# andrewdalpino/UltraZoom

Measured on AMD Instinct MI355X. Metric: upscaled MPix/sec, MewZoom-4X 1080p bf16 batched inference, higher is better.
Workload: dtype bf16; 1 GPU; MewZoom-4X 96ch/40L bf16, 16 x 1080x1920 -> 4320x7680 per GPU; global_batch=16, parallelism=batch-sharded x1, images_in_flight=0

## Files before the change

### include/mewzoom_hip.h

```cpp
#ifndef MEWZOOM_HIP_H
#define MEWZOOM_HIP_H

#include <stddef.h>
#include <stdint.h>

#ifdef __cplusplus
extern "C" {
#endif

typedef struct mz_handle mz_handle;

typedef enum mz_dtype {
    MZ_F32 = 0,
    MZ_BF16 = 1,
    MZ_F16 = 2
} mz_dtype;

typedef enum mz_status {
    MZ_OK = 0,
    MZ_ERR_INVALID_ARGUMENT = -1,
    MZ_ERR_UNKNOWN_WEIGHT = -2,
    MZ_ERR_SHAPE_MISMATCH = -3,
    MZ_ERR_MISSING_WEIGHTS = -4,
    MZ_ERR_WORKSPACE_TOO_SMALL = -5,
    MZ_ERR_HIP = -6,
    MZ_ERR_NO_DEVICE = -7
} mz_status;

typedef struct mz_config {
    int32_t upscale_ratio;
    int32_t primary_channels;
    int32_t primary_layers;
    int32_t secondary_channels;
    int32_t secondary_layers;
    int32_t tertiary_channels;
    int32_t tertiary_layers;
    int32_t quaternary_channels;
    int32_t quaternary_layers;
    int32_t hidden_ratio;
    int32_t num_deg_features;
} mz_config;


int mz_create(const mz_config* cfg, int dtype, mz_handle** out);
int mz_destroy(mz_handle* h);


int mz_num_weights(const mz_handle* h);
int mz_weight_info(const mz_handle* h, int index, const char** name, int64_t shape[4]);

int mz_set_weight(mz_handle* h, const char* name, const float* dev_f32, const int64_t* shape, int ndim,
                  void* hip_stream);

int mz_weights_complete(const mz_handle* h);


int mz_workspace_bytes(const mz_handle* h, int B, int H, int W, int max_images_in_flight, size_t* bytes);

int mz_forward(mz_handle* h, const void* x, void* out_sr, float* out_qa, int B, int H, int W, int clamp,
               void* workspace, size_t workspace_bytes, int max_images_in_flight, void* hip_stream);

int mz_forward_u8(mz_handle* h, const uint8_t* x, uint8_t* out_sr, float* out_qa, int B, int H, int W,
                  void* workspace, size_t workspace_bytes, int max_images_in_flight, void* hip_stream);

typedef struct mz_image_view {
    void*   data;
    int64_t stride[4];
} mz_image_view;

int mz_forward_view(mz_handle* h, const mz_image_view* x, const mz_image_view* out, float* out_qa,
                    int B, int H, int W, int clamp, int elem, const int32_t window[4],
                    void* workspace, size_t workspace_bytes, int max_images_in_flight, void* hip_stream);

int mz_padded_channels(int c);

int mz_op_conv(int dtype, int kind, const void* in0, const void* in1, const float* w_dev_f32, float alpha,
               void* out, int B, int H, int W, int cin, int cout, int Hout, int Wout, int silu,
               void* hip_stream);
int mz_op_stem(int dtype, const void* x, const float* w_dev_f32, const float* b_dev_f32, void* out, int B,
               int H, int W, int cout, void* hip_stream);
int mz_op_final(int dtype, const void* feat, const void* img, const float* w_dev_f32, void* out, int B, int H,
                int W, int cin, int R, int clamp, void* hip_stream);

int mz_op_conv_mix(int dtype, const void* hid, const void* x, const float* w2_dev_f32, const float* wmix_dev_f32, float alpha,
                   void* out, int B, int H, int W, int cin, int cout, void* hip_stream);

int mz_op_conv_film(int dtype, const void* in0, const float* w_dev_f32, const float* gamma_dev_f32,
                    const float* beta_dev_f32, void* out, int B, int H, int W, int cin, int cout, int silu,
                    void* hip_stream);

#define MZ_METRIC_SLOTS 16
#define MZ_METRIC_PSNR 1
#define MZ_METRIC_SSIM 2
#define MZ_METRIC_VIF 4
int mz_metrics_workspace_bytes(int B, int H, int W, int which, size_t* bytes);
int mz_metrics(const mz_image_view* pred, const mz_image_view* target, int elem, int B, int H, int W, int which,
               double data_range, double sigma_n_sq, double* out_dev, void* workspace, size_t workspace_bytes, void* hip_stream);

int mz_luma(const mz_image_view* x, const mz_image_view* out, int elem, int B, int H, int W, int standard, int clamp,
            void* hip_stream);
int mz_metrics_luma_workspace_bytes(int B, int H, int W, int which, size_t* bytes);
int mz_metrics_luma(const mz_image_view* pred, const mz_image_view* target, int elem, int B, int H, int W, int which, int standard,
                    double data_range, double sigma_n_sq, double* out_dev, void* workspace, size_t workspace_bytes, void* hip_stream);
int mz_debug_luma_coeffs(int standard, double out[4]);

#define MZ_RESIZE_BICUBIC 0
#define MZ_RESIZE_BILINEAR 1
int mz_resize_workspace_bytes(int Hin, int Win, int Hout, int Wout, int filter, size_t* bytes);
int mz_resize(const mz_image_view* x, const mz_image_view* out, int elem, int B, int Hin, int Win, int Hout, int Wout,
              int filter, int clamp, const int32_t window[4], void* workspace, size_t workspace_bytes, void* hip_stream);
int mz_debug_resize_taps(int n_in, int n_out, int filter, int i, int* first, double* w, int cap);

#define MZ_INTERP_NEAREST  0
#define MZ_INTERP_BILINEAR 1
#define MZ_INTERP_BICUBIC  2
int mz_interpolate(const mz_image_view* x, const mz_image_view* out, int elem, int B, int Hin, int Win,
                   int Hout, int Wout, int mode, int clamp, const int32_t window[4], void* hip_stream);
int mz_debug_interp_taps(int n_in, int n_out, int mode, int i, int idx[4], double w[4]);

int mz_blur(const mz_image_view* x, const mz_image_view* out, int elem, int B, int H, int W, double sigma, void* hip_stream);
int mz_noise(const mz_image_view* x, const mz_image_view* out, int elem, int B, int H, int W, double sigma, uint64_t seed,
             uint64_t offset, void* hip_stream);
int mz_jpeg_workspace_bytes(int B, int H, int W, size_t* bytes);
int mz_jpeg(const mz_image_view* x, const mz_image_view* out, int elem, int B, int H, int W, int quality, void* workspace,
            size_t workspace_bytes, void* hip_stream);
int mz_debug_blur_weights(double sigma, double* w, int cap);
int mz_debug_jpeg_qtable(int quality, uint8_t* luma, uint8_t* chroma);
int mz_debug_philox(const uint32_t counter[4], const uint32_t key[2], uint32_t out[4]);

int mz_dihedral_inverse(int k);
int mz_dihedral(const mz_image_view* x, const mz_image_view* out, int elem, int B, int H, int W, int k, void* hip_stream);
int mz_ensemble_workspace_bytes(int B, int H, int W, size_t* bytes);
int mz_ensemble_add(const mz_image_view* y, int elem, int B, int H, int W, int k, int first, void* workspace, size_t workspace_bytes,
                    void* hip_stream);
int mz_ensemble_finish(const mz_image_view* out, int elem, int B, int H, int W, int n, int clamp, const int32_t window[4],
                       void* workspace, size_t workspace_bytes, void* hip_stream);

const char* mz_last_error(void);
const char* mz_version(void);
double mz_flops_per_image(const mz_handle* h, int H, int W);
int mz_profile_enable(mz_handle* h, int on);
int mz_profile_dump(mz_handle* h, const char* path);
int mz_profile_read(mz_handle* h, double* conv_ms, double* conv_flops, double* conv_launches,
                    double* other_ms, double* conv_bytes);

int mz_debug_read(unsigned long long* host_dst);

const char* mz_debug_last_kernel(void);

int mz_debug_tile_list(int B, int tiles_y, int tiles_x, int ntiles, int gm, int gn, int blk4, int th, int tw, unsigned int* out, int cap);

const char* mz_debug_select(int dtype, int op, int cin, int cout, int B, int H, int W, int cus);

typedef struct mz_debug_step {
    int32_t kind, op, cin, cout, B, H, W, Hout, Wout, fused;
    int64_t off[3];
    uint64_t bytes[3];
    const char* kernel;
} mz_debug_step;

int mz_debug_schedule(const mz_handle* h, int B, int H, int W, int want_qa, int cus, mz_debug_step* out, int cap);

long long mz_debug_pack(int dtype, int op, int cin, int cout, int layout, long long* out, long long cap);

int mz_debug_store_hazard(int follower, int form, int wait_states, int dword, int iters, int blocks, unsigned int* counts_out);

#ifdef __cplusplus
}
#endif
#endif
```

### ultrazoom_amd/csrc/mz_conv3r.h

```cpp
#pragma once
#include "mz_device.h"
#include "mz_diag.h"
#include "mz_relay.h"

namespace mz {
namespace r3 {

constexpr int TH = 8;
template <int GEO> struct Geo {
    static_assert(GEO == 0 || GEO == 1, "8 x 48 or 8 x 40");
    static constexpr int TW = GEO == 0 ? 48 : 40;
    static constexpr int NPF = GEO == 0 ? 6 : 5;
    static constexpr int ROWW = TW + 2;
    static constexpr int NPIX = 10 * ROWW;
    static constexpr int DIV_MAGIC = GEO == 0 ? 1311 : 1561;
    static constexpr int X0 = 3, X1 = NPF - 3;
    static constexpr bool straddle(int pf) { return GEO == 1 && pf == 2; }
    static constexpr int dy(int pf) { return GEO == 0 ? pf / 3 : (pf >= 3 ? 1 : 0); }
    static constexpr int dx(int pf) { return GEO == 0 ? 16 * (pf % 3) : (pf < 2 ? 16 * pf : (pf == 2 ? 0 : 8 + 16 * (pf - 3))); }
};
constexpr int PLANE_ENT = 512;
constexpr int A_PLANE = PLANE_ENT * 16;
constexpr int A_SLOT = 4 * A_PLANE;
constexpr int NT = 3, NF = 6, BN = 96;
constexpr int NG = 9 * NT;
constexpr int B_BASE = 2 * A_SLOT;
constexpr int CHUNK_PIECES = 2 * NG;
constexpr int MIX_PIECES = 4 * NT * NT;

template <int NSEG> struct Seg {
    static_assert(NSEG == 2 || NSEG == 3, "two or three weight segments per chunk");
    static constexpr int start(int s) { return NSEG == 2 ? (s <= 0 ? 0 : (s == 1 ? (NG + 1) / 2 : NG)) : (NG / 3) * s; }
    static constexpr int of(int G) { return NSEG == 2 ? (G < start(1) ? 0 : 1) : G / (NG / 3); }
    static constexpr int pieces(int s) { return 2 * (start(s + 1) - start(s)); }
    static constexpr int SLOT = pieces(0) * 1024;
    static constexpr int MIX_BASE = B_BASE + 3 * SLOT;
    static constexpr int lds_bytes(bool fuse) { return fuse ? MIX_BASE + MIX_PIECES * 1024 : B_BASE + 3 * SLOT; }
};

template <int GEO, int TAP, int PF> constexpr int a_off() {
    using GG = Geo<GEO>;
    constexpr int DY = TAP / 3, DX = TAP % 3;
    return ((DY + GG::dy(PF)) * GG::ROWW + DX + GG::dx(PF)) * 16;
}

template <int NPF> struct Frag {
    u32x4 x[2][NPF];
    u32x4 w[3][2];
};

template <int N> __device__ __forceinline__ void wait_w(u32x4& w0, u32x4& w1) {
    asm volatile("s_waitcnt lgkmcnt(%2)" : "+v"(w0), "+v"(w1) : "n"(N) : "memory");
}
template <int N>
__device__ __forceinline__ void wait_wx(u32x4& w0, u32x4& w1, u32x4 (&x)[6]) {
    asm volatile("s_waitcnt lgkmcnt(%8)"
                 : "+v"(w0), "+v"(w1), "+v"(x[0]), "+v"(x[1]), "+v"(x[2]), "+v"(x[3]), "+v"(x[4]), "+v"(x[5])
                 : "n"(N)
                 : "memory");
}
template <int N>
__device__ __forceinline__ void wait_wx(u32x4& w0, u32x4& w1, u32x4 (&x)[5]) {
    asm volatile("s_waitcnt lgkmcnt(%7)"
                 : "+v"(w0), "+v"(w1), "+v"(x[0]), "+v"(x[1]), "+v"(x[2]), "+v"(x[3]), "+v"(x[4])
                 : "n"(N)
                 : "memory");
}

struct Bases {
    uint32_t a_cur, a_nxt, b_cur, b_nxt;
    uint32_t a2_cur, a2_nxt;
};
template <int GEO, int TAP, int PF> __device__ __forceinline__ u32x4 read_x(const Bases& bs, const bool next_image) {
    if constexpr (Geo<GEO>::straddle(PF)) return lds_read128<a_off<GEO, TAP, PF>()>(next_image ? bs.a2_nxt : bs.a2_cur);
    else return lds_read128<a_off<GEO, TAP, PF>()>(next_image ? bs.a_nxt : bs.a_cur);
}

template <class TT, int NSEG, int GEO, int GC, int XP, bool ZERO_C, int M>
__device__ __forceinline__ void group_mfmas(f32x4 (&acc)[Geo<GEO>::NPF][NF], Frag<Geo<GEO>::NPF>& f, const Bases& bs) {
    using GG = Geo<GEO>;
    constexpr int NPF = GG::NPF;
    if constexpr (M < 2 * NPF) {
        using S = Seg<NSEG>;
        constexpr int t = GC / 3, n = GC % 3, xp = (t + XP) & 1, xq = xp ^ 1;
        constexpr int sg = S::of(GC);
        constexpr int Gs = S::start(sg), Ge = S::start(sg + 1);
        constexpr int T = GC + 2;
        constexpr bool t_here = T < Ge;
        constexpr int t_idx = t_here ? T - Gs : T - Ge;
        constexpr int pf = (n & 1) ? NPF - 1 - M / 2 : M / 2, k = ((M / 2) & 1) ? 1 - (M & 1) : (M & 1);
        if constexpr (ZERO_C) mma16_first<TT>(acc[pf][2 * n + k], f.w[GC % 3][k], f.x[xp][pf]);
        else mma16<TT>(acc[pf][2 * n + k], f.w[GC % 3][k], f.x[xp][pf]);
        __builtin_amdgcn_sched_barrier(0);
        if constexpr (M < 2) {
            f.w[T % 3][M] = lds_read128<(2 * t_idx + M) * 1024>(t_here ? bs.b_cur : bs.b_nxt);
            __builtin_amdgcn_sched_barrier(0);
        }
        if constexpr (n < 2 && M >= 2 && M < 2 + (n == 0 ? GG::X0 : GG::X1)) {
            constexpr int pfn = GG::X0 * n + (M - 2);
            if constexpr (t + 1 < 9) f.x[xq][pfn] = read_x<GEO, (t + 1 < 9 ? t + 1 : 0), pfn>(bs, false);
            else f.x[xq][pfn] = read_x<GEO, 0, pfn>(bs, true);
            __builtin_amdgcn_sched_barrier(0);
        }
        group_mfmas<TT, NSEG, GEO, GC, XP, ZERO_C, M + 1>(acc, f, bs);
    }
}

template <class TT, int NSEG, int GEO, int G, int GE, int XP>
__device__ __forceinline__ void groups(f32x4 (&acc)[Geo<GEO>::NPF][NF], Frag<Geo<GEO>::NPF>& f, const Bases& bs, bool first) {
    using GG = Geo<GEO>;
    if constexpr (G < GE) {
        constexpr int t = G / 3, n = G % 3;
        __builtin_amdgcn_sched_barrier(0);
        if constexpr (G < 3 && XP == 0) {
            if (first) group_mfmas<TT, NSEG, GEO, G, XP, true, 0>(acc, f, bs);
            else group_mfmas<TT, NSEG, GEO, G, XP, false, 0>(acc, f, bs);
        } else {
            group_mfmas<TT, NSEG, GEO, G, XP, false, 0>(acc, f, bs);
        }
        constexpr int wn = (G + 1) % 3, xn = (t + 1 + XP) & 1;
        if constexpr (n == 2)
            wait_wx<2>(f.w[wn][0], f.w[wn][1], f.x[xn]);
        else if constexpr (n == 1)
            wait_w<GG::X0 + 2 + GG::X1>(f.w[wn][0], f.w[wn][1]);
        else
            wait_w<2 + GG::X0>(f.w[wn][0], f.w[wn][1]);
        groups<TT, NSEG, GEO, G + 1, GE, XP>(acc, f, bs, first);
    }
}

template <int H, int I> __device__ __forceinline__ void gate_reads(u32x4 (&wv)[NT], uint32_t addr) {
    if constexpr (I < NT) {
        constexpr int ks = H >> 1, part = H & 1;
        wv[I] = lds_read128<(ks * 2 * NT + part * NT + I) * 1024>(addr);
        gate_reads<H, I + 1>(wv, addr);
    }
}
template <int N> __device__ __forceinline__ void gate_wait(u32x4 (&wv)[NT]) {
    asm volatile("s_waitcnt lgkmcnt(%3)" : "+v"(wv[0]), "+v"(wv[1]), "+v"(wv[2]) : "n"(N) : "memory");
}
template <class TT, int H>
__device__ __forceinline__ void gate_halves(f32x4 (&beta)[NF], const u32x4 (&xf)[NT], const u32x4 (&zf)[NT], u32x4 (&wa)[NT],
                                            u32x4 (&wb)[NT], uint32_t addr) {
    if constexpr (H < 4 * NT) {
        constexpr int ks = H >> 1, part = H & 1;
        constexpr bool more = H + 1 < 4 * NT;
        if constexpr (more) gate_reads<H + 1, 0>(wb, addr);
        gate_wait<(more ? NT : 0)>(wa);
        __builtin_amdgcn_sched_barrier(0);
#pragma unroll
        for (int i = 0; i < NT; ++i) {
            if constexpr (ks == 0) mma16_first<TT>(beta[part * NT + i], wa[i], xf[0]);
            else if constexpr (ks < NT) mma16<TT>(beta[part * NT + i], wa[i], xf[ks]);
            else mma16<TT>(beta[part * NT + i], wa[i], zf[ks - NT]);
        }
        __builtin_amdgcn_sched_barrier(0);
        gate_halves<TT, H + 1>(beta, xf, zf, wb, wa, addr);
    }
}

}

template <class TT, int NSEG, int EPI, bool SILU, int GEO = 0, bool RAG = false>
__global__ __launch_bounds__(512) void conv3r_kernel(const ConvArgs a) {
    using namespace r3;
    using namespace relay;
    using S = Seg<NSEG>;
    using GG = Geo<GEO>;
    constexpr int NPF = GG::NPF, TW = GG::TW, ROWW = GG::ROWW, NPIX = GG::NPIX;
    constexpr int NE = NPF * NT;
    constexpr bool FUSE = EPI == EPI_FUSEDMIX;
    static_assert(!FUSE || GEO == 0, "the fused variant is built for the 8 x 48 tile");
    constexpr int B_SLOT = S::SLOT;
    static_assert(!FUSE || NSEG == 3, "the gate weights need the LDS that three weight segments leave free");
    static_assert(!RAG || (NSEG == 3 && EPI == EPI_STORE && GEO == 0), "the ragged two-chunk variant: three steps per chunk, plain stores, 8 x 48 tiles");
    extern __shared__ __attribute__((aligned(16))) char smem[];
    const int w = __builtin_amdgcn_readfirstlane((int)threadIdx.x >> 6);
    const int team = w >> 2, wq = w & 3;
    const int nchunks = a.nchunks16;
    const uint32_t lds_base = (uint32_t)(uintptr_t)(__attribute__((address_space(3))) char*)smem;

    const int xcd = blockIdx.x & 7, pos = blockIdx.x >> 3, step = gridDim.x >> 3;
    const int q = a.grid >> 3, rem = a.grid & 7;
    const int cnt = q + (xcd < rem ? 1 : 0);
    const int base = xcd < rem ? xcd * (q + 1) : rem * (q + 1) + (xcd - rem) * q;
    if (pos >= cnt) return;
    typedef uint32_t TabE __attribute__((ext_vector_type(2)));
    typedef const __attribute__((address_space(4))) TabE* TabPtr;
    const TabPtr tab = (TabPtr)(uintptr_t)a.tile_tab + base;
    struct TileE { uint32_t yx, bn; };
    auto tile_at = [&](int i) __attribute__((always_inline)) {
        const TabE e = tab[i];
        return TileE{e[0], e[1]};
    };
    int a_pos = pos;
    TileE eD, eA, eB;
    auto advance = [&]() __attribute__((always_inline)) { a_pos += step; };
    auto tile_origin = [&](const TileE e, int& b, int& y0, int& x0) __attribute__((always_inline)) {
        b = (int)(e.bn & 0xffffu);
        y0 = (int)(e.yx & 0xffffu);
        x0 = (int)(e.yx >> 16);
    };
    auto tile_nt = [](const TileE e) __attribute__((always_inline)) { return (int)(e.bn >> 16); };

    int hs = 0, us = 0;
    auto next3 = [](int v) __attribute__((always_inline)) { return v == 2 ? 0 : v + 1; };

    f32x4 acc[NPF][NF];
    Frag<NPF> f;
    RS_DECL;

    const size_t chunk_bytes = (size_t)CHUNK_PIECES * 1024;
    const long long plane_in = (long long)a.H * a.W * 16;

    uint32_t hoff[2];
    const char* img_l = nullptr;
    auto set_load_tile = [&](const TileE e) __attribute__((always_inline)) {
        int b, y0, x0;
        tile_origin(e, b, y0, x0);
        img_l = (const char*)a.in0 + (long long)b * a.p0 * plane_in;
        const int lane_ = lane_now();
        const bool interior = y0 >= 1 && x0 >= 1 && y0 + TH + 2 <= a.H && x0 + TW + 1 <= a.W;
        const uint32_t delta = ((uint32_t)(y0 - 1) * (uint32_t)a.W + (uint32_t)(x0 - 1)) * 16u;
#pragma unroll
        for (int j = 0; j < 2; ++j) {
            const int p = 64 * (wq + 4 * j) + lane_;
            const int py = (p * GG::DIV_MAGIC) >> 16, px = p - py * ROWW;
            uint32_t o = ((uint32_t)py * (uint32_t)a.W + (uint32_t)px) * 16u + delta;
            if (!interior) {
                const int gy = y0 - 1 + py, gx = x0 - 1 + px;
                const bool ok = (p < NPIX) & (gy >= 0) & (gy < a.H) & (gx >= 0) & (gx < a.W);
                o = ok ? o : 0xffffffffu;
            }
            hoff[j] = o;
        }
    };
    auto halo_piece = [&](auto i_tag, const __amdgpu_buffer_rsrc_t rsrc, char* dst, [[maybe_unused]] const bool rag = false) __attribute__((always_inline)) {
        constexpr int i = decltype(i_tag)::value;
        uint32_t off = hoff[i & 1];
        if constexpr (RAG) {
            if (rag && (i >> 1) >= a.ragged_planes) off = 0xffffffffu;
        }
        __builtin_amdgcn_raw_ptr_buffer_load_lds(rsrc, (__attribute__((address_space(3))) void*)(dst + (wq + 4 * i) * 1024), 16,
                                                 (int)off, (int)((uint32_t)(i >> 1) * (uint32_t)plane_in), 0, 0);
    };
    auto halo_rsrc = [&](int kc) __attribute__((always_inline)) {
        return __builtin_amdgcn_make_buffer_rsrc((void*)(img_l + 4LL * kc * plane_in), 0, (int)(uint32_t)(4 * plane_in), 0x00020000);
    };
    auto wseg_count = [&](int pieces) __attribute__((always_inline)) { return pieces > wq ? (pieces - wq + 3) >> 2 : 0; };
    auto wseg_piece = [&](auto i_tag, const char* s0, int mine, char* dst, uint32_t lo) __attribute__((always_inline)) {
        constexpr int i = decltype(i_tag)::value;
        if (i < mine) glds16(s0 + (size_t)wq * 1024u + (size_t)i * 4096u + lo, dst + wq * 1024 + i * 4096);
    };
    constexpr int WP = (S::pieces(0) + 3) / 4;
    auto wsrc_of = [&](int nt) __attribute__((always_inline)) {
        return (const char*)a.wpk16 + (size_t)nt * nchunks * chunk_bytes;
    };

    __amdgpu_buffer_rsrc_t orsrc;
    u32x4 xrsrc = {0u, 0u, 0u, 0u};
    uint32_t x_lane = 0;
    uint32_t e_pix = 0, eoff[NT] = {0, 0, 0};
    int e_c = 0, e_y = 0;
    [[maybe_unused]] int e_sdy = 0, e_sdx = 0;
    [[maybe_unused]] uint32_t e_soff = 0;
    auto epi_setup = [&]() __attribute__((always_inline)) {
        const int lane_ = lane_now();
        const int g = lane_ >> 4, c = lane_ & 15;
        const int lane_cu = 2 * (g & 1) + (g >> 1);
        int d_b, d_y0, d_x0;
        tile_origin(eD, d_b, d_y0, d_x0);
        const int d_nbase = tile_nt(eD) * BN;
        e_c = d_x0 + c;
        e_y = d_y0 + 2 * wq;
        if constexpr (GEO == 1) {
            e_sdy = c >= 8 ? 1 : 0;
            e_sdx = c >= 8 ? -8 : 32;
        }
        if constexpr (EPI == EPI_D2S) {
            const long long plane_o = (long long)a.Hout * a.Wout * 16;
            orsrc = __builtin_amdgcn_make_buffer_rsrc((char*)a.out + (long long)d_b * a.p_out * plane_o, 0,
                                                      (int)(uint32_t)(a.p_out * plane_o), 0x00020000);
            e_pix = ((uint32_t)(2 * e_y) * (uint32_t)a.Wout + (uint32_t)(2 * e_c)) * 16u;
            if constexpr (GEO == 1) e_soff = (uint32_t)((2 * e_sdy * a.Wout + 2 * e_sdx) * 16);
#pragma unroll
            for (int n = 0; n < NT; ++n) {
                const int nch = d_nbase + (4 * n + lane_cu) * 8;
                const int ij = nch / a.cp_out, ch = nch - ij * a.cp_out;
                eoff[n] = nch < 4 * a.cp_out
                              ? (uint32_t)(ch >> 3) * (uint32_t)plane_o + ((uint32_t)(ij >> 1) * (uint32_t)a.Wout + (uint32_t)(ij & 1)) * 16u
                              : 0xffffffffu;
            }
        } else {
            const long long plane_o = (long long)a.H * a.W * 16;
            const int p_first = d_nbase >> 3;
            const int planes = a.p_out - p_first < 4 * NT ? a.p_out - p_first : 4 * NT;
            orsrc = __builtin_amdgcn_make_buffer_rsrc((char*)a.out + ((long long)d_b * a.p_out + p_first) * plane_o, 0,
                                                      (int)(uint32_t)(planes * plane_o), 0x00020000);
            e_pix = ((uint32_t)e_y * (uint32_t)a.W + (uint32_t)e_c) * 16u;
            if constexpr (GEO == 1) e_soff = (uint32_t)((e_sdy * a.W + e_sdx) * 16);
#pragma unroll
            for (int n = 0; n < NT; ++n) eoff[n] = (uint32_t)(4 * n + lane_cu) * (uint32_t)plane_o;
            if constexpr (FUSE) {
                const unsigned long long xb = (unsigned long long)(uintptr_t)((const char*)a.in1 + (long long)d_b * a.p1 * plane_o);
                xrsrc[0] = (uint32_t)__builtin_amdgcn_readfirstlane((int)(uint32_t)xb);
                xrsrc[1] = (uint32_t)__builtin_amdgcn_readfirstlane((int)(uint32_t)((xb >> 32) & 0xffffu));
                xrsrc[2] = (uint32_t)__builtin_amdgcn_readfirstlane((int)(uint32_t)(a.p1 * plane_o));
                xrsrc[3] = 0x00020000u;
                x_lane = (uint32_t)(g >> 1) * (uint32_t)plane_o + (uint32_t)(g & 1) * 8u;
            }
        }
    };
    typedef uint32_t u32x2_ __attribute__((ext_vector_type(2)));
    u32x2_ f_xq[2][NF];
    u32x4 f_zb[NT];
    auto entry_words = [&](auto e_tag, u32x4& o) __attribute__((always_inline)) {
        constexpr int E = decltype(e_tag)::value;
        constexpr int pf = E / NT, n = E % NT;
        uint32_t pa[2], pb[2];
#pragma unroll
        for (int h = 0; h < 2; ++h) {
            float a0 = acc[pf][2 * n][2 * h], a1 = acc[pf][2 * n][2 * h + 1], b0 = acc[pf][2 * n + 1][2 * h], b1 = acc[pf][2 * n + 1][2 * h + 1];
            if constexpr (FUSE) {
                float xa[2], za[2], xc[2], zc[2];
                unpack2r<TT>(f_xq[pf & 1][2 * n][h], xa[0], xa[1]);
                unpack2r<TT>(f_zb[n][h], za[0], za[1]);
                unpack2r<TT>(f_xq[pf & 1][2 * n + 1][h], xc[0], xc[1]);
                unpack2r<TT>(f_zb[n][2 + h], zc[0], zc[1]);
                blend_pair_to(a0, a1, acc[pf][2 * n][2 * h], acc[pf][2 * n][2 * h + 1], xa[0], xa[1], za[0], za[1], a.inv_mix_scale);
                blend_pair_to(b0, b1, acc[pf][2 * n + 1][2 * h], acc[pf][2 * n + 1][2 * h + 1], xc[0], xc[1], zc[0], zc[1], a.inv_mix_scale);
            }
            if constexpr (EPI == EPI_STORE && SILU) {
                silu_pair_to(a0, a1, acc[pf][2 * n][2 * h], acc[pf][2 * n][2 * h + 1]);
                silu_pair_to(b0, b1, acc[pf][2 * n + 1][2 * h], acc[pf][2 * n + 1][2 * h + 1]);
            }
            pa[h] = pack_pair<TT>(f32x2{a0, a1});
            pb[h] = pack_pair<TT>(f32x2{b0, b1});
        }
        o = swap_packed(pa, pb);
    };
    auto epi_store = [&](auto e_tag, const u32x4& o) __attribute__((always_inline)) {
        constexpr int E = decltype(e_tag)::value;
        constexpr int pf = E / NT, n = E % NT;
        bool inside;
        uint32_t off;
        if constexpr (GG::straddle(pf)) {
            inside = e_y + e_sdy < a.H && e_c + e_sdx < a.W;
            off = e_pix + e_soff + eoff[n];
        } else {
            inside = e_y + GG::dy(pf) < a.H && e_c + GG::dx(pf) < a.W;
            if constexpr (EPI == EPI_D2S) off = e_pix + (uint32_t)(2 * GG::dy(pf)) * (uint32_t)a.Wout * 16u + (uint32_t)(2 * GG::dx(pf)) * 16u + eoff[n];
            else off = e_pix + (uint32_t)GG::dy(pf) * (uint32_t)a.W * 16u + (uint32_t)GG::dx(pf) * 16u + eoff[n];
        }
        if (!inside || eoff[n] == 0xffffffffu) off = 0xffffffffu;
        __builtin_amdgcn_raw_buffer_store_b128(o, orsrc, (int)off, 0, 0);
    };
    auto fuse_x = [&](auto pf_tag) __attribute__((always_inline)) {
        constexpr int pf = decltype(pf_tag)::value;
        const bool inside = e_y + GG::dy(pf) < a.H && e_c + GG::dx(pf) < a.W;
        const long long plane_o = (long long)a.H * a.W * 16;
        uint32_t off = e_pix + (uint32_t)GG::dy(pf) * (uint32_t)a.W * 16u + (uint32_t)GG::dx(pf) * 16u + x_lane;
        if (!inside) off = 0xffffffffu;
#pragma unroll
        for (int nf = 0; nf < NF; ++nf) {
            const uint32_t o = inside ? off + (uint32_t)(2 * nf) * (uint32_t)plane_o : 0xffffffffu;
            u32x2_& dst = f_xq[pf & 1][nf];
            const u32x4& xr = xrsrc;
            asm volatile("buffer_load_dwordx2 %0, %1, %2, 0 offen" : "=v"(dst) : "v"(o), "s"(xr) : "memory");
        }
    };
    auto x_landed = [&](auto pf_tag) __attribute__((always_inline)) {
        constexpr int pf = decltype(pf_tag)::value;
#pragma unroll
        for (int nf = 0; nf < NF; ++nf) {
            u32x2_& r = f_xq[pf & 1][nf];
            asm volatile("" : "+v"(r));
        }
    };
    auto fuse_z = [&](auto pf_tag) __attribute__((always_inline)) {
        constexpr int pf = decltype(pf_tag)::value;
#pragma unroll
        for (int m = 0; m < NT; ++m) {
            const f32x4 za = acc[pf][2 * m], zc = acc[pf][2 * m + 1];
            u32x4 q;
            q[0] = pack2r<TT>(za[0], za[1]); q[1] = pack2r<TT>(za[2], za[3]);
            q[2] = pack2r<TT>(zc[0], zc[1]); q[3] = pack2r<TT>(zc[2], zc[3]);
            asm volatile("" : "+v"(q));
            f_zb[m] = q;
        }
    };
    auto fuse_a = [&](auto pf_tag) __attribute__((always_inline)) {
        constexpr int pf = decltype(pf_tag)::value;
        if constexpr (pf + 1 < NPF) fuse_x(ic<(pf + 1 < NPF ? pf + 1 : 0)>{});
        fuse_z(pf_tag);
    };
    auto fuse_c = [&](auto pf_tag) __attribute__((always_inline)) {
        constexpr int pf = decltype(pf_tag)::value;
        const int lane_ = lane_now();
        const uint32_t mix_lane = lds_base + S::MIX_BASE + lane_ * 16;
        u32x4 xb[NT];
#pragma unroll
        for (int m = 0; m < NT; ++m) xb[m] = u32x4{f_xq[pf & 1][2 * m][0], f_xq[pf & 1][2 * m][1], f_xq[pf & 1][2 * m + 1][0], f_xq[pf & 1][2 * m + 1][1]};
        u32x4 wa[NT], wb[NT];
        gate_reads<0, 0>(wa, mix_lane);
        gate_halves<TT, 0>(acc[pf], xb, f_zb, wa, wb, mix_lane);
        gate_settle();
    };
    auto entry_whole = [&](auto e_tag) __attribute__((always_inline)) {
        if constexpr (decltype(e_tag)::value < NE) {
            u32x4 o;
            entry_words(e_tag, o);
            epi_store(e_tag, o);
        }
    };

    auto prime = [&](int wslot, int aslot) __attribute__((always_inline)) {
        const int lane_ = lane_now();
        const int g = lane_ >> 4, c = lane_ & 15;
        Bases pb;
        pb.a_cur = pb.a_nxt = lds_base + aslot * A_SLOT + g * A_PLANE + ((2 * wq) * ROWW + c) * 16;
        pb.a2_cur = pb.a2_nxt = pb.a_cur + (uint32_t)((c >= 8 ? ROWW - 8 : 32) * 16);
        pb.b_cur = pb.b_nxt = 0;
        const uint32_t bb = lds_base + B_BASE + wslot * B_SLOT + lane_ * 16;
        f.x[0][0] = read_x<GEO, 0, 0>(pb, false);
        f.x[0][1] = read_x<GEO, 0, 1>(pb, false);
        f.x[0][2] = read_x<GEO, 0, 2>(pb, false);
        f.x[0][3] = read_x<GEO, 0, 3>(pb, false);
        f.x[0][4] = read_x<GEO, 0, 4>(pb, false);
        if constexpr (NPF > 5) f.x[0][NPF - 1] = read_x<GEO, 0, NPF - 1>(pb, false);
        f.w[0][0] = lds_read128<0 * 1024>(bb);
        f.w[0][1] = lds_read128<1 * 1024>(bb);
        f.w[1][0] = lds_read128<2 * 1024>(bb);
        f.w[1][1] = lds_read128<3 * 1024>(bb);
        wait_wx<0>(f.w[0][0], f.w[0][1], f.x[0]);
        wait_w<0>(f.w[1][0], f.w[1][1]);
    };

    const char* wA = nullptr;
    const char* wB = nullptr;
    bool okB = false;
    auto loader_step = [&](auto wk_tag, auto es_tag, auto en_tag, auto sg_tag, auto last_tag, int k) __attribute__((always_inline)) {
        constexpr int WK = decltype(wk_tag)::value;
        constexpr int ES = decltype(es_tag)::value, EN = WK == 0 ? 0 : decltype(en_tag)::value, sg = decltype(sg_tag)::value;
        constexpr bool last = decltype(last_tag)::value != 0;
        [[maybe_unused]] constexpr int rs_c = 1 + (EN > 0 ? 2 : 0) + (sg == 0 ? 0 : 1);
        static_assert(EN <= 3, "three output registers");
        constexpr int VM_AFTER0 = WK == 1 ? EN : (WK == 2 ? (ES + 1 < NPF ? NF : 0) : (WK == 4 ? EN * NT : 0));
        constexpr int VM_AFTER = VM_AFTER0 + (NSEG == 3 && sg == 0 ? 8 : 0);
        RS_BEGIN();
        if constexpr (WK == 2 && ES == 0) fuse_x(ic<0>{});
        if constexpr (WK == 3) x_landed(ic<ES>{});
        constexpr bool HALO_LATE = NSEG == 3;
        auto halo_image = [&]() __attribute__((always_inline)) {
            const __amdgpu_buffer_rsrc_t h_rsrc = halo_rsrc(last ? 0 : k + 1);
            uint32_t h_off = (uint32_t)(us ^ 1) * (uint32_t)A_SLOT;
            asm volatile("" : "+s"(h_off));
            char* const h_dst = smem + h_off;
            const bool rag = RAG && !last && k + 2 == nchunks;
            halo_piece(ic<0>{}, h_rsrc, h_dst, rag); halo_piece(ic<1>{}, h_rsrc, h_dst, rag); halo_piece(ic<2>{}, h_rsrc, h_dst, rag);
            halo_piece(ic<3>{}, h_rsrc, h_dst, rag); halo_piece(ic<4>{}, h_rsrc, h_dst, rag); halo_piece(ic<5>{}, h_rsrc, h_dst, rag);
            halo_piece(ic<6>{}, h_rsrc, h_dst, rag); halo_piece(ic<7>{}, h_rsrc, h_dst, rag);
        };
        if constexpr (sg == 0 && !HALO_LATE) {
            if (!last || okB) halo_image();
        }
        {
            constexpr bool same = sg + 2 < NSEG;
            constexpr int qs = same ? sg + 2 : sg + 2 - NSEG;
            const char* wsrc;
            bool w_ok = true;
            if constexpr (same) wsrc = wA + (size_t)k * chunk_bytes;
            else if constexpr (!last) wsrc = wA + (size_t)(k + 1) * chunk_bytes;
            else { wsrc = wB; w_ok = okB; }
            wsrc += (size_t)(2 * S::start(qs)) * 1024;
            const int w_pieces = w_ok ? wseg_count(S::pieces(qs)) : 0;
            char* const w_dst = smem + B_BASE + (hs >= 1 ? hs - 1 : 2) * B_SLOT;
            const uint32_t lo = (uint32_t)lane_now() * 16u;
            wseg_piece(ic<0>{}, wsrc, w_pieces, w_dst, lo); wseg_piece(ic<1>{}, wsrc, w_pieces, w_dst, lo); wseg_piece(ic<2>{}, wsrc, w_pieces, w_dst, lo);
            wseg_piece(ic<3>{}, wsrc, w_pieces, w_dst, lo); wseg_piece(ic<4>{}, wsrc, w_pieces, w_dst, lo);
            if constexpr (WP > 5) wseg_piece(ic<5>{}, wsrc, w_pieces, w_dst, lo);
            if constexpr (WP > 6) wseg_piece(ic<6>{}, wsrc, w_pieces, w_dst, lo);
            static_assert(WP <= 7, "seven weight pieces per wave and step");
        }
        if constexpr (sg == 0 && HALO_LATE) halo_image();
        __builtin_amdgcn_sched_barrier(0);
        asm volatile("" ::: "memory");
        RS_LAP(4 * rs_c);
        if constexpr (WK == 1) {
            u32x4 o0, o1, o2;
            if constexpr (EN > 0) entry_words(ic<ES>{}, o0);
            if constexpr (EN > 1) entry_words(ic<ES + 1>{}, o1);
            if constexpr (EN > 2) entry_words(ic<ES + 2>{}, o2);
            if constexpr (EN > 0) epi_store(ic<ES>{}, o0);
            if constexpr (EN > 1) epi_store(ic<ES + 1>{}, o1);
            if constexpr (EN > 2) epi_store(ic<ES + 2>{}, o2);
        } else if constexpr (WK == 2) {
            static_assert(WK != 2 || EN == 1, "one pixel fragment per chunk");
            fuse_a(ic<ES>{});
        } else if constexpr (WK == 3) {
            fuse_c(ic<ES>{});
        } else if constexpr (WK == 4) {
            entry_whole(ic<3 * ES>{}); entry_whole(ic<3 * ES + 1>{}); entry_whole(ic<3 * ES + 2>{});
        }
        RS_FENCE();
        RS_LAP(4 * rs_c + 1);
        if constexpr (sg == NSEG - 1) {
            if constexpr (last) {
                if constexpr (FUSE) zero_acc(acc);
                prime(next3(hs), us ^ 1);
            } else {
                if (k + 2 == nchunks && okB) {
                    set_load_tile(eB);
                }
            }
        }
        __builtin_amdgcn_sched_barrier(0);
        RS_LAP(sg == NSEG - 1 ? (last ? 26 : 25) : 4 * rs_c + 1);
        wait_vmcnt<VM_AFTER>();
        RS_LAP(4 * rs_c + 2);
        __builtin_amdgcn_s_barrier();
        RS_LAP(4 * rs_c + 3);
        RS_COUNT(20 + rs_c);
        hs = next3(hs);
        if constexpr (sg == NSEG - 1) us ^= 1;
    };
    auto loader_chunk = [&](auto e0_tag, auto n0_tag, auto n1_tag, auto last_tag, int k) __attribute__((always_inline)) {
        constexpr int E0 = decltype(e0_tag)::value < NE ? decltype(e0_tag)::value : NE;
        constexpr int N0 = decltype(n0_tag)::value < NE - E0 ? decltype(n0_tag)::value : NE - E0;
        constexpr int N1 = decltype(n1_tag)::value < NE - E0 - N0 ? decltype(n1_tag)::value : NE - E0 - N0;
        if constexpr (NSEG == 2) {
            loader_step(ic<(N0 > 0)>{}, ic<E0>{}, ic<N0>{}, ic<0>{}, last_tag, k);
            loader_step(ic<(N1 > 0)>{}, ic<E0 + N0>{}, ic<N1>{}, ic<1>{}, last_tag, k);
        } else {
            constexpr int N1a = N1 / 2, N1b = N1 - N1a;
            loader_step(ic<(N0 > 0)>{}, ic<E0>{}, ic<N0>{}, ic<0>{}, last_tag, k);
            loader_step(ic<(N1a > 0)>{}, ic<E0 + N0>{}, ic<N1a>{}, ic<1>{}, last_tag, k);
            loader_step(ic<(N1b > 0)>{}, ic<E0 + N0 + N1a>{}, ic<N1b>{}, ic<2>{}, last_tag, k);
        }
    };
    auto fuse_chunk = [&](auto p0_tag, auto g_tag, auto last_tag, int k) __attribute__((always_inline)) {
        static_assert(!FUSE || NSEG == 3, "the fused variant runs three steps per chunk");
        loader_step(ic<2>{}, p0_tag, g_tag, ic<0>{}, last_tag, k);
        loader_step(ic<3>{}, p0_tag, g_tag, ic<1>{}, last_tag, k);
        loader_step(ic<4>{}, p0_tag, g_tag, ic<NSEG - 1>{}, last_tag, k);
    };
    auto plain_chunks = [&](int k0) __attribute__((always_inline)) {
        for (int k = k0; k + 1 < nchunks; ++k) loader_chunk(ic<0>{}, ic<0>{}, ic<0>{}, ic<0>{}, k);
        loader_chunk(ic<0>{}, ic<0>{}, ic<0>{}, ic<1>{}, nchunks - 1);
    };
    auto loader_phase = [&](auto epi_tag) __attribute__((always_inline)) {
        constexpr bool DO_EPI = decltype(epi_tag)::value != 0;
        wA = wsrc_of(tile_nt(eA));
        okB = a_pos + step < cnt;
        wB = wsrc_of(tile_nt(okB ? eB : eA));
        const TileE eA2 = tile_at(a_pos + 2 * step), eB2 = tile_at(a_pos + 3 * step);
        if constexpr (DO_EPI) {
            RS_BEGIN();
            set_load_tile(eA);
            epi_setup();
            RS_FENCE();
            RS_LAP(27);
            if constexpr (RAG) {
                loader_chunk(ic<0>{}, ic<3>{}, ic<6>{}, ic<0>{}, 0);
                loader_chunk(ic<9>{}, ic<3>{}, ic<6>{}, ic<1>{}, 1);
            } else if constexpr (FUSE) {
                fuse_chunk(ic<0>{}, ic<1>{}, ic<0>{}, 0);
                fuse_chunk(ic<1>{}, ic<1>{}, ic<0>{}, 1);
                fuse_chunk(ic<2>{}, ic<1>{}, ic<0>{}, 2);
                fuse_chunk(ic<3>{}, ic<1>{}, ic<0>{}, 3);
                fuse_chunk(ic<4>{}, ic<1>{}, ic<0>{}, 4);
                if (nchunks == 6) {
                    fuse_chunk(ic<5>{}, ic<1>{}, ic<1>{}, 5);
                } else {
                    fuse_chunk(ic<5>{}, ic<1>{}, ic<0>{}, 5);
                    plain_chunks(6);
                }
            } else if (nchunks >= 6) {
                loader_chunk(ic<0>{}, ic<1>{}, ic<2>{}, ic<0>{}, 0);
                loader_chunk(ic<3>{}, ic<1>{}, ic<2>{}, ic<0>{}, 1);
                loader_chunk(ic<6>{}, ic<1>{}, ic<2>{}, ic<0>{}, 2);
                loader_chunk(ic<9>{}, ic<1>{}, ic<2>{}, ic<0>{}, 3);
                loader_chunk(ic<12>{}, ic<1>{}, ic<2>{}, ic<0>{}, 4);
                if (nchunks == 6) {
                    loader_chunk(ic<15>{}, ic<1>{}, ic<2>{}, ic<1>{}, 5);
                } else {
                    loader_chunk(ic<15>{}, ic<1>{}, ic<2>{}, ic<0>{}, 5);
                    plain_chunks(6);
                }
            } else {
                constexpr int F3 = NSEG == 3 ? 2 : 3;
                loader_chunk(ic<0>{}, ic<F3>{}, ic<6 - F3>{}, ic<0>{}, 0);
                loader_chunk(ic<6>{}, ic<F3>{}, ic<6 - F3>{}, ic<0>{}, 1);
                if (nchunks == 3) {
                    loader_chunk(ic<12>{}, ic<F3>{}, ic<6 - F3>{}, ic<1>{}, 2);
                } else {
                    loader_chunk(ic<12>{}, ic<F3>{}, ic<6 - F3>{}, ic<0>{}, 2);
                    plain_chunks(3);
                }
            }
        } else {
            plain_chunks(0);
        }
        eD = eB; eA = eA2; eB = eB2;
        asm volatile("" ::"s"(eA.yx), "s"(eA.bn), "s"(eB.yx), "s"(eB.bn));
    };

    auto compute_phase = [&]() __attribute__((always_inline)) {
        const int lane_ = lane_now();
        const int g = lane_ >> 4, c = lane_ & 15;
        const uint32_t a_lane = lds_base + g * A_PLANE + ((2 * wq) * ROWW + c) * 16;
        Bases bs;
        bs.a_cur = a_lane + us * A_SLOT;
        bs.a_nxt = a_lane + (us ^ 1) * A_SLOT;
        const uint32_t a_str = (uint32_t)((c >= 8 ? ROWW - 8 : 32) * 16);
        bs.a2_cur = bs.a_cur + a_str;
        bs.a2_nxt = bs.a_nxt + a_str;
        const uint32_t bl = lds_base + B_BASE + lane_ * 16;
        uint32_t b0 = bl + hs * B_SLOT, b1 = bl + next3(hs) * B_SLOT, b2 = bl + next3(next3(hs)) * B_SLOT;
        bs.b_cur = b0;
        bs.b_nxt = b1;
        auto step_tail = [&]() __attribute__((always_inline)) {
            __builtin_amdgcn_s_barrier();
            const uint32_t u_ = b0; b0 = b1; b1 = b2; b2 = u_;
            bs.b_cur = b0; bs.b_nxt = b1;
        };
        auto chunk = [&](auto xp_tag, bool first) __attribute__((always_inline)) {
            constexpr int XP = decltype(xp_tag)::value;
            groups<TT, NSEG, GEO, S::start(0), S::start(1), XP>(acc, f, bs, first);
            step_tail();
            groups<TT, NSEG, GEO, S::start(1), S::start(2), XP>(acc, f, bs, false);
            step_tail();
            if constexpr (NSEG == 3) {
                groups<TT, NSEG, GEO, S::start(2), S::start(3), XP>(acc, f, bs, false);
                step_tail();
            }
            const uint32_t v_ = bs.a_cur; bs.a_cur = bs.a_nxt; bs.a_nxt = v_;
            if constexpr (GEO == 1) { const uint32_t v2_ = bs.a2_cur; bs.a2_cur = bs.a2_nxt; bs.a2_nxt = v2_; }
        };
        RS_BEGIN();
        int kc = 0;
        for (;;) {
            chunk(ic<0>{}, !FUSE && kc == 0);
            if (++kc >= nchunks) break;
            chunk(ic<1>{}, false);
            if (++kc >= nchunks) break;
        }
        asm volatile("s_waitcnt lgkmcnt(0)"
                     : "+v"(f.x[0][0]), "+v"(f.x[0][1]), "+v"(f.x[0][2]), "+v"(f.x[0][3]), "+v"(f.x[0][4]), "+v"(f.x[0][NPF - 1]),
                       "+v"(f.x[1][0]), "+v"(f.x[1][1]), "+v"(f.x[1][2]), "+v"(f.x[1][3]), "+v"(f.x[1][4]), "+v"(f.x[1][NPF - 1])
                     :
                     : "memory");
        asm volatile("" : "+v"(f.w[0][0]), "+v"(f.w[0][1]), "+v"(f.w[1][0]), "+v"(f.w[1][1]), "+v"(f.w[2][0]), "+v"(f.w[2][1]));
        RS_LAP(0);
        RS_COUNT(1);
        const int adv = (NSEG * nchunks) % 3;
        hs = hs + adv >= 3 ? hs + adv - 3 : hs + adv;
        us ^= nchunks & 1;
    };
    auto final_fuse_pf = [&](auto pf_tag) __attribute__((always_inline)) {
        constexpr int pf = decltype(pf_tag)::value;
        fuse_x(pf_tag);
        fuse_z(pf_tag);
        wait_vmcnt<0>();
        x_landed(pf_tag);
        fuse_c(pf_tag);
        entry_whole(ic<3 * pf>{}); entry_whole(ic<3 * pf + 1>{}); entry_whole(ic<3 * pf + 2>{});
    };
    auto final_epilogue = [&]() __attribute__((always_inline)) {
        epi_setup();
        if constexpr (FUSE) {
            final_fuse_pf(ic<0>{}); final_fuse_pf(ic<1>{}); final_fuse_pf(ic<2>{}); final_fuse_pf(ic<3>{}); final_fuse_pf(ic<4>{}); final_fuse_pf(ic<5>{});
        } else {
            entry_whole(ic<0>{}); entry_whole(ic<1>{}); entry_whole(ic<2>{}); entry_whole(ic<3>{}); entry_whole(ic<4>{}); entry_whole(ic<5>{});
            entry_whole(ic<6>{}); entry_whole(ic<7>{}); entry_whole(ic<8>{}); entry_whole(ic<9>{}); entry_whole(ic<10>{}); entry_whole(ic<11>{});
            entry_whole(ic<12>{}); entry_whole(ic<13>{}); entry_whole(ic<14>{}); entry_whole(ic<15>{}); entry_whole(ic<16>{}); entry_whole(ic<17>{});
        }
    };

    if (team == 1) {
        eA = tile_at(a_pos);
        eB = tile_at(a_pos + step);
        eD = eA;
        wA = wsrc_of(tile_nt(eA));
        set_load_tile(eA);
        {
            const __amdgpu_buffer_rsrc_t r0 = halo_rsrc(0);
            halo_piece(ic<0>{}, r0, smem); halo_piece(ic<1>{}, r0, smem); halo_piece(ic<2>{}, r0, smem); halo_piece(ic<3>{}, r0, smem);
            halo_piece(ic<4>{}, r0, smem); halo_piece(ic<5>{}, r0, smem); halo_piece(ic<6>{}, r0, smem); halo_piece(ic<7>{}, r0, smem);
            const char* s1 = wA + (size_t)(2 * S::start(1)) * 1024;
            const uint32_t lo = (uint32_t)lane_now() * 16u;
            char* d0 = smem + B_BASE;
            char* d1 = smem + B_BASE + B_SLOT;
            wseg_piece(ic<0>{}, wA, wseg_count(S::pieces(0)), d0, lo); wseg_piece(ic<1>{}, wA, wseg_count(S::pieces(0)), d0, lo); wseg_piece(ic<2>{}, wA, wseg_count(S::pieces(0)), d0, lo);
            wseg_piece(ic<3>{}, wA, wseg_count(S::pieces(0)), d0, lo); wseg_piece(ic<4>{}, wA, wseg_count(S::pieces(0)), d0, lo); wseg_piece(ic<5>{}, wA, wseg_count(S::pieces(0)), d0, lo);
            wseg_piece(ic<6>{}, wA, wseg_count(S::pieces(0)), d0, lo);
            wseg_piece(ic<0>{}, s1, wseg_count(S::pieces(1)), d1, lo); wseg_piece(ic<1>{}, s1, wseg_count(S::pieces(1)), d1, lo); wseg_piece(ic<2>{}, s1, wseg_count(S::pieces(1)), d1, lo);
            wseg_piece(ic<3>{}, s1, wseg_count(S::pieces(1)), d1, lo); wseg_piece(ic<4>{}, s1, wseg_count(S::pieces(1)), d1, lo); wseg_piece(ic<5>{}, s1, wseg_count(S::pieces(1)), d1, lo);
            wseg_piece(ic<6>{}, s1, wseg_count(S::pieces(1)), d1, lo);
        }
        if constexpr (FUSE) {
            const int lane_ = lane_now();
            const char* msrc = (const char*)a.wmix16 + (uint32_t)lane_ * 16u;
#pragma unroll
            for (int i = 0; i < MIX_PIECES / 4; ++i) glds16(msrc + (size_t)(wq + 4 * i) * 1024, smem + S::MIX_BASE + (wq + 4 * i) * 1024);
        }
        wait_vmcnt<0>();
        __builtin_amdgcn_s_barrier();
        if constexpr (FUSE) zero_acc(acc);
        loader_phase(ic<0>{});
        advance();
        if (a_pos >= cnt) { RS_DUMP(); return; }
    } else {
        eD = tile_at(a_pos);
        eA = tile_at(a_pos + step);
        eB = tile_at(a_pos + 2 * step);
        asm volatile("" ::"s"(eD.yx), "s"(eD.bn), "s"(eA.yx), "s"(eA.bn), "s"(eB.yx), "s"(eB.bn));
        __builtin_amdgcn_s_barrier();
        if constexpr (FUSE) zero_acc(acc);
        prime(0, 0);
    }
    for (;;) {
        compute_phase();
        advance();
        if (a_pos >= cnt) {
            RS_BEGIN();
            final_epilogue();
            RS_LAP(2);
            RS_DUMP();
            return;
        }
        loader_phase(ic<1>{});
        advance();
        if (a_pos >= cnt) { RS_DUMP(); return; }
    }
}

}
```

### ultrazoom_amd/csrc/mz_conv3r.hip

```cpp
#include "mz_conv3r.h"

#ifndef MZ_R_NSEG
#define MZ_R_NSEG 3
#endif

namespace mz {

template <class TT, int NSEG, int EPI, bool SILU = false, int GEO = 0, bool RAG = false> static hipError_t r_launch(const ConvArgs& a, hipStream_t s) {
    constexpr size_t lds = r3::Seg<NSEG>::lds_bytes(EPI == EPI_FUSEDMIX);
    return launch_lds<conv3r_kernel<TT, NSEG, EPI, SILU, GEO, RAG>>(a.persist, 512, lds, a, s);
}
template <class TT> static hipError_t r_epi(const ConvArgs& a, hipStream_t s) {
    if (a.ragged_planes) {
        if (a.nchunks16 != 2 || a.ragged_planes < 1 || a.ragged_planes > 3 || a.epi != EPI_STORE || !a.silu || a.geo != 0) return hipErrorInvalidValue;
        return r_launch<TT, 3, EPI_STORE, true, 0, true>(a, s);
    }
    if (a.nchunks16 < 3) return hipErrorInvalidValue;
    if (a.geo == 1) {
        switch (a.epi) {
            case EPI_STORE: return a.silu ? r_launch<TT, MZ_R_NSEG, EPI_STORE, true, 1>(a, s) : r_launch<TT, MZ_R_NSEG, EPI_STORE, false, 1>(a, s);
            case EPI_D2S: return r_launch<TT, MZ_R_NSEG, EPI_D2S, false, 1>(a, s);
            default: return hipErrorInvalidValue;
        }
    }
    switch (a.epi) {
        case EPI_STORE: return a.silu ? r_launch<TT, MZ_R_NSEG, EPI_STORE, true>(a, s) : r_launch<TT, MZ_R_NSEG, EPI_STORE, false>(a, s);
        case EPI_D2S: return r_launch<TT, MZ_R_NSEG, EPI_D2S>(a, s);
        case EPI_FUSEDMIX: return a.wmix16 ? r_launch<TT, 3, EPI_FUSEDMIX>(a, s) : hipErrorInvalidValue;
        default: return hipErrorInvalidValue;
    }
}

hipError_t launch_conv3r(int dtype, const ConvArgs& a, hipStream_t s) {
    if (a.persist <= 0 || (a.persist & 7) || a.nchunks16 < 2 || a.geo < 0 || a.geo > 1) return hipErrorInvalidValue;
    switch (dtype) {
        case DT_BF16: return r_epi<TBF16>(a, s);
        case DT_F16: return r_epi<TF16>(a, s);
        default: return hipErrorInvalidValue;
    }
}

}
```

### ultrazoom_amd/csrc/mz_debug.cpp

```cpp
#include <cstdarg>
#include <cstdio>

#include "mz_host.h"
#include "mz_pack.h"

using namespace mz;

static thread_local char g_err[512] = "";
thread_local const char* mz::g_last_kernel = "";
int mz::fail(int code, const char* fmt, ...) {
    va_list ap;
    va_start(ap, fmt);
    vsnprintf(g_err, sizeof(g_err), fmt, ap);
    va_end(ap);
    return code;
}
extern "C" const char* mz_last_error(void) { return g_err; }
extern "C" const char* mz_debug_last_kernel(void) { return g_last_kernel; }

int mz::device_cus() {
    static int known[kMaxDevices];
    int n = 0, dev = 0;
    if (hipGetDeviceCount(&n) != hipSuccess || n <= 0) return fail(MZ_ERR_NO_DEVICE, "no HIP device visible");
    if (hipGetDevice(&dev) != hipSuccess || dev < 0 || dev >= kMaxDevices) return fail(MZ_ERR_NO_DEVICE, "bad current device");
    if (!known[dev]) {
        int c = 0;
        if (hipDeviceGetAttribute(&c, hipDeviceAttributeMultiprocessorCount, dev) != hipSuccess) c = 0;
        known[dev] = c / 8 * 8 + 1;
    }
    return known[dev] - 1;
}

extern "C" int mz_debug_read(unsigned long long* host_dst) {
    unsigned long long* b = debug_buffer();
    if (!b) return -1;
    return hipMemcpy(host_dst, b, 16 * 64 * 8 * sizeof(unsigned long long), hipMemcpyDeviceToHost) == hipSuccess ? 0 : -6;
}

extern "C" int mz_debug_tile_list(int B, int tiles_y, int tiles_x, int ntiles, int gm, int gn, int blk4, int th, int tw, unsigned int* out, int cap) {
    if (B < 1 || tiles_x < 1 || tiles_y < 1 || ntiles < 1 || gm < 1 || gn < 1 || th < 1 || tw < 1 || !out || cap < 0) return MZ_ERR_INVALID_ARGUMENT;
    const int mtiles = B * tiles_x * tiles_y;
    std::vector<uint32_t> t;
    tile_list(group_walk(tiles_x, tiles_y, mtiles, ntiles, std::min(gm, mtiles), std::min(gn, ntiles), blk4 ? 1 : 0), th, tw, t);
    const int n = (int)(t.size() / 2);
    for (int i = 0; i < n && i < cap; ++i) { out[2 * i] = t[2 * i]; out[2 * i + 1] = t[2 * i + 1]; }
    return n;
}

template <class T> static T refused(T nothing, const Refusal& r) { fail(r); return nothing; }

extern "C" const char* mz_debug_select(int dtype, int op, int cin, int cout, int B, int H, int W, int cus) {
    const char* const none = nullptr;
    if ((dtype != MZ_F32 && dtype != MZ_BF16 && dtype != MZ_F16) || cin < 1 || cout < 1 || B < 1 || H < 1 || W < 1 || cus < 0)
        return refused(none, refuse(MZ_ERR_INVALID_ARGUMENT, "bad arguments"));
    if (op == 5 && dtype != DT_BF16 && dtype != DT_F16)
        return refused(none, refuse(MZ_ERR_INVALID_ARGUMENT, "the FiLM epilogue is implemented for bf16 / fp16"));
    if (op == 8) return refused(none, refuse(MZ_ERR_INVALID_ARGUMENT, "bad op %d", op));
    const Knobs k = read_knobs();
    BlockPlan b;
    Refusal why;
    const LayerPlan* c = plan_debug_layer(b, dtype, op, cin, cout, &why);
    if (!c) return refused(none, why);
    if (op == 7) return kernel_name(choose_mix(k, dtype, *c, B, H, W, cus));
    Conv3Call call;
    switch (op) {
        case 0: call = conv1_call(*c, nullptr, nullptr, B, H, W); break;
        case 2: call = d2s_call(*c, nullptr, nullptr, B, H, W, 2 * H, 2 * W); break;
        case 3: call = head_call(*c, nullptr, nullptr, B, H, W); break;
        case 5: call = film_call(*c, nullptr, nullptr, B, H, W, 0); break;
        case 6: call = conv2_call(k, b, nullptr, nullptr, B, H, W); break;
        default: call = plain_call(*c, nullptr, nullptr, B, H, W); break;
    }
    const KernelChoice ch = choose_conv3(k, dtype, call, cus);
    return ch.ok ? kernel_name(ch) : refused(none, refuse(MZ_ERR_INVALID_ARGUMENT, "%s", ch.why));
}

extern "C" long long mz_debug_pack(int dtype, int op, int cin, int cout, int layout, long long* out, long long cap) {
    if ((dtype != MZ_F32 && dtype != MZ_BF16 && dtype != MZ_F16) || cin < 1 || cout < 1 || layout < 0 || layout >= PK_COUNT || cap < 0 ||
        (cap > 0 && !out))
        return refused(-1LL, refuse(MZ_ERR_INVALID_ARGUMENT, "bad arguments"));
    BlockPlan b;
    Refusal why;
    const LayerPlan* c = plan_debug_layer(b, dtype, op, cin, cout, &why);
    if (!c) return refused(-1LL, why);
    if (!c->has(layout)) return refused(-1LL, refuse(MZ_ERR_INVALID_ARGUMENT, "the layer has no packing %d", layout));
    const PackArgs p = pack_args(*c, layout, dtype, nullptr, nullptr);
    const long long n = (long long)(packed_bytes(p.taps, p.frags, p.ntiles, p.nchunks) / dtype_size(dtype));
    for (long long i = 0; i < n && i < cap; ++i) out[i] = dtype == DT_F32 ? pack_source<4>(p, i) : pack_source<2>(p, i);
    return n;
}
extern "C" const char* mz_version(void) { return "mewzoom_hip 0.1 (gfx950)"; }

extern "C" double mz_flops_per_image(const mz_handle* h, int H, int W) {
    if (!h) return 0.0;
    Plan p;
    make_plan(h->dims, 1, H, W, p);
    long long macs = 0;
    for (const auto& st : make_schedule(h->model, h->dims, p, h->ctx.knobs,  true, h->cfg.upscale_ratio, 0)) macs += step_macs(st);
    return 2.0 * (double)macs;
}

extern "C" int mz_debug_schedule(const mz_handle* h, int B, int H, int W, int want_qa, int cus, mz_debug_step* out, int cap) {
    if (!h || cap < 0 || (cap > 0 && !out) || cus < 0) return fail(MZ_ERR_INVALID_ARGUMENT, "bad arguments");
    if (B <= 0 || H < 8 || W < 8) return fail(MZ_ERR_INVALID_ARGUMENT, "need B >= 1 and H, W >= 8 (got %d, %d, %d)", B, H, W);
    const Knobs& k = h->ctx.knobs;
    const int dtype = h->dims.dtype;
    Plan p;
    make_plan(h->dims, B, H, W, p);
    const auto steps = make_schedule(h->model, h->dims, p, k, want_qa != 0, h->cfg.upscale_ratio, 0);
    static const int role_op[] = {-1, 0, 6, 4, 2, 3};
    for (size_t i = 0; i < steps.size() && i < (size_t)cap; ++i) {
        const Step<ConvW>& st = steps[i];
        mz_debug_step& d = out[i];
        d.kind = st.kind;
        d.op = st.kind == ST_MIX ? 7 : role_op[st.role];
        d.cin = st.cin; d.cout = st.cout;
        d.B = st.B; d.H = st.H; d.W = st.W; d.Hout = st.Hout; d.Wout = st.Wout;
        d.fused = st.fused;
        const BufRef* bufs[3] = {&st.in, &st.in1, &st.out};
        for (int j = 0; j < 3; ++j) {
            d.off[j] = bufs[j]->where == BUF_WS ? (long long)bufs[j]->off : bufs[j]->where;
            d.bytes[j] = bufs[j]->bytes;
        }
        d.kernel = nullptr;
        if (st.kind == ST_MIX) d.kernel = kernel_name(choose_mix(k, dtype, *st.layer, st.B, st.H, st.W, cus));
        if (st.kind == ST_CONV3) d.kernel = kernel_name(choose_conv3(k, dtype, step_call(k, st, nullptr, nullptr, nullptr), cus));
    }
    return (int)steps.size();
}
```

### ultrazoom_amd/csrc/mz_kernels.h

```cpp
#pragma once
#include <hip/hip_runtime.h>
#include <stddef.h>
#include <stdint.h>

namespace mz {

enum DType : int { DT_F32 = 0, DT_BF16 = 1, DT_F16 = 2 };

inline int dtype_size(int dt) { return dt == DT_F32 ? 4 : 2; }
inline int chunk_channels(int dt) { return dt == DT_F32 ? 8 : 16; }
inline int pad16(int c) { return (c + 15) / 16 * 16; }

enum ConvMode : int { MODE_CONV3 = 0, MODE_GEMM1 = 1, MODE_C3W16 = 2, MODE_C3W8 = 3 };
enum SrcKind : int { SRC_PLAIN = 0, SRC_CONCAT = 1, SRC_CRUSH = 2, SRC_MIXF = 3  };
enum Epilogue : int {
    EPI_STORE = 0,
    EPI_D2S = 1,
    EPI_MIX = 2,
    EPI_FINAL = 3,
    EPI_FUSEDMIX = 4,
};

struct ConvArgs {
    const void* in0;
    const void* in1;
    const void* wpk;
    void* out;
    const void* zero;
    const void* img;
    const void* wmix;
    int mix_pieces;
    int x_via_lds;
    int B, H, W;
    int Ho, Wo;
    int p0, p1;
    int p_out;
    int nchunks;
    int nchunks_real;
    int nchunks0;
    int src;
    int ntiles;
    int mtiles;
    int tiles_x, tiles_y;
    int gm, gn;
    int grid;
    int groups_m;
    float inv_gsz, inv_groups_m, inv_gn, inv_tpi, inv_tiles_x;
    int blk4;
    float inv_bsz;
    uint32_t mg_gsz, mg_groups_m, mg_gn, mg_tpi, mg_tiles_x, mg_bsz;
    int epi;
    int silu;
    int cp_out;
    int Hout, Wout;
    float mix_scale;
    float inv_mix_scale;
    int R;
    int Hi, Wi;
    int clamp;
    int io_u8;
    int persist;
    int s16;
    const void* wpk16;
    int nchunks16;
    const void* tile_tab;
    int ragged_planes;
    int geo;
    const void* wmix16;
    const float* film_gamma;
    const float* film_beta;
    int use_glds;
    unsigned long long* dbg;
    int view;
    long long vin[4], vout[4];
    int win_y0, win_x0, win_h, win_w;
};

struct ImageViews {
    long long in[4], out[4];
    int y0, x0, h, w;
};

inline int choose_nt(int n_padded) {
    const int order[4] = {3, 2, 4, 1};
    int best = 1, best_n = 1 << 30;
    for (int i = 0; i < 4; ++i) {
        const int bn = 32 * order[i];
        const int padded = (n_padded + bn - 1) / bn * bn;
        if (padded < best_n) {
            best_n = padded;
            best = order[i];
        }
    }
    return best;
}

enum Kernel : int {
    K_CONV256,
    K_CONV3W,
    K_CONV3P,
    K_CONV3S,
    K_CONV3R,
    K_CONV3T,
    K_MIX16,
    K_MIX16B,
};
constexpr int kMaxDevices = 64;
inline bool walk_ok(const ConvArgs& a) {
    return a.mtiles > 0 && a.ntiles > 0 && a.gm > 0 && a.gn > 0 && a.grid > 0 && a.grid < (1 << 24);
}
hipError_t launch_conv256(int dtype, int mode, int nt, const ConvArgs& a, hipStream_t s);
hipError_t launch_conv3w(int dtype, int mode, int nt, const ConvArgs& a, hipStream_t s);
hipError_t launch_conv3p(int dtype, int mode, int nt, const ConvArgs& a, hipStream_t s);
hipError_t launch_conv3s(int dtype, int mode, int nt, const ConvArgs& a, hipStream_t s);
hipError_t launch_mix16(int dtype, const ConvArgs& a, hipStream_t s);
hipError_t launch_mix16b(int dtype, const ConvArgs& a, hipStream_t s, int workgroups);
hipError_t launch_conv3r(int dtype, const ConvArgs& a, hipStream_t s);
hipError_t launch_conv3t(int dtype, const ConvArgs& a, hipStream_t s);

enum OutMap : int { OUT_PLAIN = 0, OUT_D2S = 1, OUT_FINAL = 2 };
enum PackLayout : int {
    PK_MAIN = 0,
    PK_CONV16,
    PK_MIX16,
    PK_GATE16,
    PK_MIX16B,
    PK_GATE16R,
    PK_CONV16T,
    PK_GATE16T,
    PK_COUNT
};
struct PackArgs {
    const float* w;
    void* dst;
    int dtype;
    int layout;
    int cout, cin, kh, kw;
    int taps;
    int frags, ntiles, nchunks;
    int out_map;
    int cq, cq_p;
    int in_map;
    int c0, cp0, c1;
};
inline size_t packed_bytes(int taps, int nt, int ntiles, int nchunks) { return (size_t)ntiles * nchunks * taps * nt * 1024; }
hipError_t launch_pack(const PackArgs& a, hipStream_t s);

hipError_t launch_pack_stem(const float* w, const float* b, float* dst, int c, int cp, hipStream_t s);
hipError_t launch_stem(int dtype, const void* x, const float* w4, void* out, int B, int H, int W, int cp,
                       hipStream_t s, int u8 = 0, const long long* vin = nullptr);
hipError_t launch_zero_border(int dtype, void* t, int B, int Hout, int Wout, int cp, int Hv, int Wv,
                              hipStream_t s);
hipError_t launch_qa_reduce(int dtype, const void* feat, const float* bias, float* qa, int B, int P, int cp,
                            int F, hipStream_t s);
hipError_t launch_fill_zero(void* p, size_t bytes, hipStream_t s);

}
```

### ultrazoom_amd/csrc/mz_plan.h

```cpp
#pragma once
#include <stdlib.h>

#include <algorithm>
#include <vector>

#include "mz_geo.h"

namespace mz {

struct Knobs {
    bool wide = true;
    bool fuse = true;
    bool s16 = true;
    bool fuse16 = true;
    bool mix16b = true;
    int persist = -1;
    int kpad_pct = 12;
    int blk4 = 1;
    int r = 1;
    int r2 = 1;
    int t = 1;
};
inline Knobs read_knobs() {
    Knobs k;
    k.wide = getenv("MZ_NO_WIDE") == nullptr;
    k.fuse = getenv("MZ_NO_FUSE") == nullptr;
    k.s16 = getenv("MZ_NO_S16") == nullptr;
    k.fuse16 = getenv("MZ_NO_FUSE16") == nullptr;
    k.mix16b = getenv("MZ_NO_MIX16B") == nullptr;
    k.r = getenv("MZ_NO_R") == nullptr;
    k.t = getenv("MZ_NO_T") == nullptr;
    k.r2 = getenv("MZ_NO_R2") == nullptr;
    k.blk4 = getenv("MZ_NO_BLK4") == nullptr;
    if (const char* e = getenv("MZ_KPAD_PCT")) k.kpad_pct = atoi(e);
    if (getenv("MZ_NO_PERSIST") != nullptr) k.persist = 0;
    else if (const char* e = getenv("MZ_PERSIST_WGS")) { const int n = atoi(e) / 8 * 8; k.persist = n > 0 ? n : 0; }
    return k;
}

struct LayerPlan {
    int cout = 0, cin = 0, kh = 0, kw = 0;
    int mode = MODE_CONV3, taps = 9, nt = 1, ntiles = 1, nchunks = 1, nchunks_real = 1;
    int out_map = OUT_PLAIN, cq = 0, cq_p = 0;
    int in_map = SRC_PLAIN, c0 = 0, cp0 = 0, c1 = 0;
    int n_logical_padded = 0;
    int nchunks32 = 0;
    unsigned layouts = 0;
    bool has(int layout) const { return layouts >> layout & 1u; }
};

struct PackShape { int frags, ntiles, nchunks; };
inline PackShape pack_shape(const LayerPlan& c, int layout) {
    switch (layout) {
        case PK_MAIN: return {c.nt, c.ntiles, c.nchunks};
        case PK_CONV16: return {2 * c.nt, c.ntiles, c.nchunks32};
        case PK_MIX16: case PK_MIX16B: return {12, c.cout / 192, 2 * c.cout / 32};
        case PK_GATE16: case PK_GATE16R: return {2 * c.nt, 1, c.nchunks32 + c.nt};
        case PK_CONV16T: return {3, 1, c.nchunks32};
        default: return {3, 1, 3};
    }
}
inline size_t pack_bytes(const LayerPlan& c, int layout) {
    const PackShape sh = pack_shape(c, layout);
    return packed_bytes(c.taps, sh.frags, sh.ntiles, sh.nchunks);
}
inline PackArgs pack_args(const LayerPlan& c, int layout, int dtype, const float* w_dev, void* dst) {
    const PackShape sh = pack_shape(c, layout);
    PackArgs p;
    p.w = w_dev; p.dst = dst; p.dtype = dtype; p.layout = layout;
    p.cout = c.cout; p.cin = c.cin; p.kh = c.kh; p.kw = c.kw;
    p.taps = c.taps; p.frags = sh.frags; p.ntiles = sh.ntiles; p.nchunks = sh.nchunks;
    p.out_map = c.out_map; p.cq = c.cq; p.cq_p = c.cq_p;
    p.in_map = c.in_map; p.c0 = c.c0; p.cp0 = c.cp0; p.c1 = c.c1;
    return p;
}

inline void plan_conv(LayerPlan& c, int dtype, int mode, int cout, int cin, int kh, int kw, int out_map, int in_map, int c0, int c1) {
    const int ck = chunk_channels(dtype);
    c.cout = cout; c.cin = cin; c.kh = kh; c.kw = kw;
    c.mode = mode;
    c.taps = mode == MODE_CONV3 ? 9 : 1;
    c.out_map = out_map;
    c.in_map = in_map;
    if (out_map == OUT_D2S) {
        c.cq = cout / 4;
        c.cq_p = pad16(c.cq);
        c.n_logical_padded = 4 * c.cq_p;
    } else if (out_map == OUT_FINAL) {
        c.n_logical_padded = 16;
    } else {
        c.n_logical_padded = pad16(cout);
    }
    c.nt = choose_nt(c.n_logical_padded);
    c.ntiles = (c.n_logical_padded + 32 * c.nt - 1) / (32 * c.nt);
    if (in_map == SRC_PLAIN) {
        c.c0 = cin; c.cp0 = pad16(cin); c.c1 = 0;
        c.nchunks = c.cp0 / ck;
    } else if (in_map == SRC_CONCAT) {
        c.c0 = c0; c.cp0 = pad16(c0); c.c1 = c1;
        c.nchunks = (c.cp0 + pad16(c1)) / ck;
    } else {
        c.c0 = cin; c.cp0 = pad16(cin); c.c1 = 0;
        c.nchunks = 4 * c.cp0 / ck;
    }
    c.nchunks_real = c.nchunks;
    if (mode == MODE_GEMM1) {
        const int S = gemm1_chunks_per_stage();
        c.nchunks = (c.nchunks + S - 1) / S * S;
    }
    c.nchunks32 = (c.cp0 + 31) / 32;
    c.layouts = 1u << PK_MAIN;
    const bool s16 = dtype != DT_F32;
    if (mode == MODE_CONV3 && s16 && in_map == SRC_PLAIN && out_map != OUT_FINAL && c.nt <= 3) c.layouts |= 1u << PK_CONV16;
    if (mode == MODE_CONV3 && s16 && in_map == SRC_PLAIN && out_map == OUT_PLAIN && c.n_logical_padded == 48 && c.cp0 % 32 == 0)
        c.layouts |= 1u << PK_CONV16T;
    if (mode == MODE_GEMM1 && s16 && in_map == SRC_CONCAT && cout % 192 == 0 && c0 == cout && c1 == cout) {
        c.layouts |= 1u << PK_MIX16;
        if (cout == 192) c.layouts |= 1u << PK_MIX16B;
    }
}

inline void plan_mixf(LayerPlan& f, int dtype, const LayerPlan& conv2) {
    const int c = conv2.cout;
    f.cout = c; f.cin = 2 * c; f.kh = f.kw = 1;
    f.mode = MODE_GEMM1; f.taps = 1;
    f.nt = conv2.nt; f.ntiles = 1;
    f.out_map = OUT_PLAIN; f.in_map = SRC_MIXF;
    f.c0 = c; f.cp0 = pad16(c); f.c1 = c;
    const int zg = dtype == DT_F32 ? 4 : 2;
    f.nchunks = f.nchunks_real = f.cp0 / chunk_channels(dtype) + f.nt * zg;
    f.nchunks32 = (f.cp0 + 31) / 32;
    f.layouts = 1u << PK_MAIN;
    if (dtype != DT_F32) {
        f.layouts |= 1u << PK_GATE16;
        if (f.nt == 3) f.layouts |= 1u << PK_GATE16R;
        if (f.cp0 == 48) f.layouts |= 1u << PK_GATE16T;
    }
}

template <class Layer> struct Block {
    Layer conv1, conv2, mix;
    Layer mixf;
    bool fused = false;
    float alpha = 0.f;
};
using BlockPlan = Block<LayerPlan>;

template <class Layer> void plan_block(Block<Layer>& b, int dtype, int c, int hidden) {
    plan_conv(b.conv1, dtype, MODE_CONV3, hidden, c, 3, 3, OUT_PLAIN, SRC_PLAIN, 0, 0);
    plan_conv(b.conv2, dtype, MODE_CONV3, c, hidden, 3, 3, OUT_PLAIN, SRC_PLAIN, 0, 0);
    plan_conv(b.mix, dtype, MODE_GEMM1, c, 2 * c, 1, 1, OUT_PLAIN, SRC_CONCAT, c, c);
    b.fused = b.conv2.ntiles == 1 && b.conv2.nt <= 3;
    if (b.fused) plan_mixf(b.mixf, dtype, b.conv2);
}

struct ModelDims { int dtype, ch[4], hidden_ratio, nhead, num_deg_features; };

template <class Layer> struct Model {
    int enc[4], dec[4];
    std::vector<Block<Layer>> enc_blocks[4], dec_blocks[4], head_blocks;
    Layer crush[3], up[3], skipmix[3];
    float skip_alpha[3] = {0, 0, 0};
    std::vector<Layer> head_up;
    Layer qa_conv;
};

template <class Layer> void plan_model(Model<Layer>& m, const ModelDims& d, const int layers[4]) {
    const int* ch = d.ch;
    auto plan_blocks = [&](std::vector<Block<Layer>>& blocks, int n, int c) {
        blocks = std::vector<Block<Layer>>(n);
        for (auto& b : blocks) plan_block(b, d.dtype, c, d.hidden_ratio * c);
    };
    for (int l = 0; l < 4; ++l) {
        m.enc[l] = (layers[l] + 1) / 2;
        m.dec[l] = layers[l] / 2;
        plan_blocks(m.enc_blocks[l], m.enc[l], ch[l]);
        plan_blocks(m.dec_blocks[3 - l], m.dec[l], ch[l]);
    }
    for (int l = 0; l < 3; ++l)
        plan_conv(m.crush[l], d.dtype, MODE_GEMM1, ch[l + 1], ch[l], 2, 2, OUT_PLAIN, SRC_CRUSH, 0, 0);
    plan_conv(m.qa_conv, d.dtype, MODE_CONV3, d.num_deg_features, ch[3], 3, 3, OUT_PLAIN, SRC_PLAIN, 0, 0);
    for (int i = 0; i < 3; ++i) {
        const int cin = ch[3 - i], cout = ch[2 - i];
        plan_conv(m.up[i], d.dtype, MODE_CONV3, 4 * cout, cin, 3, 3, OUT_D2S, SRC_PLAIN, 0, 0);
        plan_conv(m.skipmix[i], d.dtype, MODE_GEMM1, cout, 2 * cout, 1, 1, OUT_PLAIN, SRC_CONCAT, cout, cout);
    }
    plan_blocks(m.head_blocks, d.nhead, ch[0]);
    m.head_up = std::vector<Layer>(d.nhead);
    for (int i = 0; i < d.nhead; ++i) {
        const bool last = i == d.nhead - 1;
        plan_conv(m.head_up[i], d.dtype, MODE_CONV3, 4 * (last ? 3 : ch[0]), ch[0], 3, 3, last ? OUT_FINAL : OUT_D2S, SRC_PLAIN, 0, 0);
    }
}

struct Plan {
    int nb;
    int hs[4], ws[4];
    size_t R[4][3], HID[4], Z[4], U[3];
    size_t HR[3][2], HHID[3], HZ[3];
    size_t QA;
    size_t total;
};

inline size_t align_up(size_t v) { return (v + 255) & ~(size_t)255; }

inline void make_plan(const ModelDims& m, int nb, int H, int W, Plan& p) {
    const size_t sz = dtype_size(m.dtype);
    const int hr = m.hidden_ratio;
    size_t off = 0;
    auto take = [&](size_t bytes) {
        size_t o = off;
        off += align_up(bytes);
        return o;
    };
    p.nb = nb;
    p.hs[0] = H; p.ws[0] = W;
    for (int i = 1; i < 4; ++i) { p.hs[i] = p.hs[i - 1] / 2; p.ws[i] = p.ws[i - 1] / 2; }
    for (int l = 0; l < 4; ++l) {
        const size_t px = (size_t)nb * p.hs[l] * p.ws[l];
        const size_t c = px * pad16(m.ch[l]) * sz;
        for (int k = 0; k < 3; ++k) p.R[l][k] = take(c);
        p.HID[l] = take(px * pad16(hr * m.ch[l]) * sz);
        p.Z[l] = take(c);
        if (l < 3) p.U[l] = take(c);
    }
    for (int j = 1; j < m.nhead; ++j) {
        const size_t px = (size_t)nb * ((size_t)H << j) * ((size_t)W << j);
        const size_t c = px * pad16(m.ch[0]) * sz;
        p.HR[j][0] = take(c);
        p.HR[j][1] = take(c);
        p.HHID[j] = take(px * pad16(hr * m.ch[0]) * sz);
        p.HZ[j] = take(c);
    }
    p.QA = take((size_t)nb * p.hs[3] * p.ws[3] * pad16(m.num_deg_features) * sz);
    p.total = off;
}

inline int default_micro_batch(const ModelDims& m, int B, int H, int W, int requested) {
    if (requested > 0) return std::min(B, requested);
    Plan p;
    make_plan(m, 1, H, W, p);
    const size_t budget = (size_t)48 << 30;
    int nb = (int)std::max<size_t>(1, budget / std::max<size_t>(1, p.total));
    return std::max(1, std::min(B, nb));
}

}
```

### ultrazoom_amd/csrc/mz_runner.h

```cpp
#pragma once
#include <cmath>
#include <cstring>
#include <map>
#include <utility>

#include "mz_err.h"
#include "mz_select.h"

namespace mz {

struct DevBuf {
    void* p = nullptr;
    DevBuf() = default;
    DevBuf(DevBuf&& o) noexcept : p(o.p) { o.p = nullptr; }
    ~DevBuf() {
        if (p) (void)hipFree(p);
    }
    hipError_t alloc(size_t bytes) { return p ? hipSuccess : hipMalloc(&p, bytes); }
};

struct ConvW : LayerPlan {
    DevBuf packed[PK_COUNT];
};
using BlockW = Block<ConvW>;
inline const ConvW& weights(const LayerPlan* c) { return *static_cast<const ConvW*>(c); }

inline int pack_conv(ConvW& c, int dtype, const float* w_dev, hipStream_t s) {
    for (int l = 0; l < PK_COUNT; ++l) {
        if (!c.has(l)) continue;
        HIPCHK(c.packed[l].alloc(pack_bytes(c, l)));
        HIPCHK(launch_pack(pack_args(c, l, dtype, w_dev, c.packed[l].p), s));
    }
    return MZ_OK;
}

struct ProfRec {
    hipEvent_t a, b;
    double flops, bytes;
    int kind, B, H, W, cin, cout, nt, ntiles, mtiles, n_fast;
};

struct LaunchCtx {
    DevBuf zero_page;
    Knobs knobs = read_knobs();
    std::map<std::vector<int>, std::pair<DevBuf, int>> tile_tabs;
    bool prof = false;
    std::vector<ProfRec> recs;
    size_t recs_used = 0;
    int init(hipStream_t s) {
        HIPCHK(zero_page.alloc(4096));
        HIPCHK(hipMemsetAsync(zero_page.p, 0, 4096, s));
        return MZ_OK;
    }
    ~LaunchCtx() {
        for (auto& r : recs) {
            (void)hipEventDestroy(r.a);
            (void)hipEventDestroy(r.b);
        }
    }
};

inline unsigned long long* debug_buffer() {
    static unsigned long long* buf = nullptr;
    static bool tried = false;
    if (!tried) {
        tried = true;
        if (getenv("MZ_DEBUG_STAMPS")) {
            if (hipMalloc((void**)&buf, 16 * 64 * 8 * sizeof(unsigned long long)) != hipSuccess) buf = nullptr;
            else (void)hipMemset(buf, 0, 16 * 64 * 8 * sizeof(unsigned long long));
        }
    }
    return buf;
}

inline float inv_sigmoid(float alpha) {
    const float v = 1.0f + std::exp(-alpha);
    return std::isfinite(v) ? v : 3.402823466e+38f;
}

struct Runner {
    LaunchCtx& ctx;
    hipStream_t s;
    int dtype;
    int rc = MZ_OK;
    const Knobs knobs = ctx.knobs;
    int io_u8 = 0;
    int cus = std::max(0, device_cus());

    ProfRec* prof_begin(int kind, const ConvArgs& a, const LayerPlan& c, double flops, double bytes) {
        if (!ctx.prof) return nullptr;
        if (ctx.recs_used == ctx.recs.size()) {
            ProfRec n;
            if (hipEventCreate(&n.a) != hipSuccess || hipEventCreate(&n.b) != hipSuccess) return nullptr;
            ctx.recs.push_back(n);
        }
        ProfRec* r = &ctx.recs[ctx.recs_used++];
        r->flops = flops; r->bytes = bytes;
        r->kind = kind; r->B = a.B; r->H = a.H; r->W = a.W; r->cin = c.cin; r->cout = c.cout; r->nt = c.nt; r->ntiles = a.ntiles;
        r->mtiles = a.mtiles; r->n_fast = a.gm * 1000 + a.gn;
        (void)hipEventRecord(r->a, s);
        return r;
    }

    int check(hipError_t e, const char* what) {
        if (e != hipSuccess && rc == MZ_OK) rc = hip_rc(e, what);
        return rc;
    }

    void base_args(ConvArgs& a, const ConvW& c, const void* in0, void* out, int B, int H, int W, int cp_out, const Walk& w) {
        memset(&a, 0, sizeof(a));
        a.wpk = c.packed[PK_MAIN].p;
        a.zero = ctx.zero_page.p;
        a.dbg = debug_buffer();
        a.nchunks = c.nchunks;
        a.nchunks_real = c.nchunks_real;
        a.in0 = in0; a.out = out;
        a.B = B; a.H = H; a.W = W; a.Ho = H; a.Wo = W;
        a.p0 = c.cp0 * dtype_size(dtype) / 16;
        a.cp_out = cp_out;
        a.p_out = a.cp_out * dtype_size(dtype) / 16;
        put_walk(a, w);
    }

    void tile_table(ConvArgs& a, const Walk& w, int th, int tw, int wgs) {
        const int pad = 4 * ((wgs > 256 ? wgs : 256) / 8) + 8;
        const std::vector<int> key = {th, tw, a.B, w.tiles_x, w.tiles_y, w.ntiles, w.gm, w.gn, w.grid, w.blk4, pad};
        auto it = ctx.tile_tabs.find(key);
        if (it == ctx.tile_tabs.end()) {
            std::vector<uint32_t> t;
            t.reserve(2 * ((size_t)w.mtiles * w.ntiles + pad));
            tile_list(w, th, tw, t);
            const int n = (int)(t.size() / 2);
            t.resize(t.size() + 2 * (size_t)pad, 0u);
            DevBuf d;
            if (check(d.alloc(t.size() * 4), "tile table")) return;
            if (check(hipMemcpy(d.p, t.data(), t.size() * 4, hipMemcpyHostToDevice), "tile table upload")) return;
            it = ctx.tile_tabs.emplace(key, std::make_pair(std::move(d), n)).first;
        }
        a.tile_tab = it->second.first.p;
        a.grid = it->second.second;
    }

    hipError_t launch_kernel(const KernelChoice& ch, const ConvArgs& a, int nt) {
        switch (ch.kernel) {
            case K_CONV256: return launch_conv256(dtype, ch.mode, nt, a, s);
            case K_CONV3W: return launch_conv3w(dtype, ch.mode, nt, a, s);
            case K_CONV3P: return launch_conv3p(dtype, ch.mode, nt, a, s);
            case K_CONV3S: return launch_conv3s(dtype, ch.mode, nt, a, s);
            case K_CONV3R: return launch_conv3r(dtype, a, s);
            case K_CONV3T: return launch_conv3t(dtype, a, s);
            case K_MIX16: return launch_mix16(dtype, a, s);
            case K_MIX16B: return launch_mix16b(dtype, a, s, ch.persist);
        }
        return hipErrorInvalidValue;
    }
    void launch(const KernelChoice& ch, const ConvArgs& a, int nt, ProfRec* r, const char* what = nullptr) {
        if (!what) what = g_last_kernel = kernel_name(ch);
        check(launch_kernel(ch, a, nt), what);
        if (r) (void)hipEventRecord(r->b, s);
    }

    void conv3(const Conv3Call& k) {
        if (rc) return;
        const KernelChoice ch = choose_conv3(knobs, dtype, k, cus);
        if (!ch.ok) { rc = fail(MZ_ERR_INVALID_ARGUMENT, "%s", ch.why); return; }
        const ConvW& c = weights(k.c);
        const int B = k.B, H = k.H, W = k.W;
        const double sz = dtype_size(dtype);
        const double px = (double)B * H * W;
        const int tiles_x = (W + ch.tw - 1) / ch.tw, tiles_y = (H + ch.th - 1) / ch.th;
        const Walk w = pick_order(tiles_x, tiles_y, B * tiles_x * tiles_y, c.ntiles, (double)pack_bytes(c, PK_MAIN), px * c.cp0 * sz, knobs);
        ConvArgs a;
        base_args(a, c, k.in, k.out, B, H, W, k.epi == EPI_D2S ? c.cq_p : pad16(c.cout), w);
        a.src = SRC_PLAIN;
        a.epi = k.epi; a.silu = k.silu;
        a.Hout = k.Hout; a.Wout = k.Wout;
        a.img = k.img; a.R = k.R; a.clamp = k.clamp;
        if (k.epi == EPI_FINAL) { a.Hi = k.Hout / k.R; a.Wi = k.Wout / k.R; a.io_u8 = io_u8; }
        if (k.epi == EPI_FINAL && k.views) {
            a.view = 1;
            for (int i = 0; i < 4; ++i) { a.vin[i] = k.views->in[i]; a.vout[i] = k.views->out[i]; }
            a.win_y0 = k.views->y0; a.win_x0 = k.views->x0; a.win_h = k.views->h; a.win_w = k.views->w;
        }
        const bool fused = ch.fused;
        if (fused) {
            a.in1 = k.xin;
            a.p1 = pad16(c.cout) * dtype_size(dtype) / 16;
            a.wmix = weights(k.mixf).packed[PK_MAIN].p;
            a.mix_pieces = k.mixf->nchunks * k.mixf->nt;
            const int slot = ch.mode == MODE_C3W16 ? stage_bytes<MODE_C3W16>(c.nt) : stage_bytes<MODE_C3W8>(c.nt);
            const int ncx = a.p1 / 2;
            a.x_via_lds = (a.mix_pieces * 1024 + 8 * ncx * 1024 <= 2 * slot) ? 1 : 0;
            a.mix_scale = 1.0f / (1.0f + std::exp(-k.alpha));
            a.inv_mix_scale = inv_sigmoid(k.alpha);
        }
        a.geo = ch.geo;
        a.ragged_planes = ch.ragged_planes;
        if (ch.layout != PK_MAIN) {
            a.wpk16 = c.packed[ch.layout].p;
            a.nchunks16 = pack_shape(c, ch.layout).nchunks;
            if (fused) a.wmix16 = weights(k.mixf).packed[ch.gate].p;
        }
        if (ch.tile_list) tile_table(a, w, ch.th, ch.tw, ch.persist);
        if (rc) return;
        a.persist = std::min((a.grid + 7) / 8 * 8, ch.persist);
        a.film_gamma = k.gamma; a.film_beta = k.beta;
        const double flops = 2.0 * px * 9.0 * c.cin * c.cout + (fused ? 2.0 * px * 2.0 * c.cout * c.cout : 0.0);
        const double bytes = px * (c.cin + c.cout) * sz + 9.0 * c.cin * c.cout * sz + (fused ? px * c.cout * sz : 0.0);
        launch(ch, a, c.nt, prof_begin(0, a, c, flops, bytes));
    }

    void mix(const ConvW& c, float alpha, const void* x, const void* z, void* out, int B, int H, int W) {
        if (rc) return;
        const KernelChoice ch = choose_mix(knobs, dtype, c, B, H, W, cus);
        const int sz = dtype_size(dtype);
        const long long npix = (long long)B * H * W;
        const bool mix16 = ch.layout != PK_MAIN;
        const PackShape sh = pack_shape(c, ch.layout);
        ConvArgs a;
        base_args(a, c, x, out, B, H, W, pad16(c.cout),
                  pick_order(0, 0, (int)((npix + 255) / 256), sh.ntiles, (double)pack_bytes(c, PK_MAIN),
                             (double)npix * (c.cp0 + pad16(c.c1)) * sz, knobs, mix16 ? 32 : 64));
        a.in1 = z; a.p1 = pad16(c.c1) * sz / 16;
        a.nchunks0 = c.cp0 / chunk_channels(dtype);
        a.src = SRC_CONCAT;
        a.epi = EPI_MIX;
        a.mix_scale = 1.0f / (1.0f + std::exp(-alpha));
        a.inv_mix_scale = inv_sigmoid(alpha);
        if (mix16) {
            a.wpk16 = c.packed[ch.layout].p;
            a.nchunks16 = sh.nchunks;
        }
        launch(ch, a, c.nt, prof_begin(1, a, c, 2.0 * (double)npix * c.cin * c.cout, (double)npix * 3.0 * c.cout * sz));
    }

    void crush(const ConvW& c, const void* in, void* out, int B, int H, int W) {
        if (rc) return;
        const double sz = dtype_size(dtype);
        const long long npix = (long long)B * (H / 2) * (W / 2);
        ConvArgs a;
        base_args(a, c, in, out, B, H, W, pad16(c.cout),
                  pick_order(0, 0, (int)((npix + 255) / 256), c.ntiles, (double)pack_bytes(c, PK_MAIN), (double)B * H * W * c.cp0 * sz, knobs, 64));
        a.Ho = H / 2; a.Wo = W / 2;
        a.nchunks0 = c.cp0 / chunk_channels(dtype);
        a.src = SRC_CRUSH;
        a.epi = EPI_STORE;
        ProfRec* r = prof_begin(2, a, c, 2.0 * (double)npix * 4.0 * c.cin * c.cout, ((double)B * H * W * c.cin + (double)npix * c.cout) * sz);
        KernelChoice ch;
        ch.ok = true; ch.kernel = K_CONV256; ch.mode = MODE_GEMM1;
        launch(ch, a, c.nt, r, "crush launch");
    }
};

}
```

### ultrazoom_amd/csrc/mz_select.h

```cpp
#pragma once
#include <math.h>

#include <vector>

#include "mz_plan.h"
#include "mz_view_check.h"

namespace mz {

struct Walk {
    int tiles_x = 0, tiles_y = 0;
    int mtiles = 0, ntiles = 0;
    int gm = 1, gn = 1, groups_m = 0, grid = 0;
    int blk4 = 0;
    float inv_gsz = 1.f, inv_groups_m = 1.f, inv_gn = 1.f, inv_tpi = 1.f, inv_tiles_x = 1.f, inv_bsz = 1.f;
};

inline Walk group_walk(int tiles_x, int tiles_y, int mtiles, int ntiles, int gm, int gn, int blk4) {
    Walk w;
    w.tiles_x = tiles_x; w.tiles_y = tiles_y; w.mtiles = mtiles; w.ntiles = ntiles;
    w.gm = gm; w.gn = gn; w.blk4 = blk4;
    w.groups_m = (mtiles + gm - 1) / gm;
    w.grid = (int)((long long)w.groups_m * ((ntiles + gn - 1) / gn) * gm * gn);
    w.inv_gsz = 1.0f / (float)(gm * gn);
    w.inv_groups_m = 1.0f / (float)w.groups_m;
    w.inv_gn = 1.0f / (float)gn;
    if (tiles_x > 0) {
        w.inv_tpi = 1.0f / (float)(tiles_x * tiles_y);
        w.inv_tiles_x = 1.0f / (float)tiles_x;
        w.inv_bsz = 1.0f / (float)(4 * tiles_x);
    }
    return w;
}

inline Walk pick_order(int tiles_x, int tiles_y, int mtiles, int ntiles, double weight_bytes, double act_bytes, const Knobs& k,
                       int resident_per_xcd = 32) {
    int best_gm = mtiles, best_gn = 1;
    double best = 1e300;
    for (int gn = 1; gn <= ntiles; ++gn) {
        if (gn > resident_per_xcd) break;
        if (ntiles % gn != 0 && gn != ntiles) continue;
        int gm = resident_per_xcd / gn;
        if (gm < 1) gm = 1;
        if (gm > mtiles) gm = mtiles;
        const double groups_n = ceil((double)ntiles / gn), groups_m = ceil((double)mtiles / gm);
        const double traffic = act_bytes * groups_n + weight_bytes * groups_m;
        if (traffic < best) { best = traffic; best_gm = gm; best_gn = gn; }
    }
    return group_walk(tiles_x, tiles_y, mtiles, ntiles, best_gm, best_gn, k.blk4 && tiles_x > 0 && 4 * tiles_x < 65536 ? 1 : 0);
}

inline void put_walk(ConvArgs& a, const Walk& w) {
    a.tiles_x = w.tiles_x; a.tiles_y = w.tiles_y; a.mtiles = w.mtiles; a.ntiles = w.ntiles;
    a.gm = w.gm; a.gn = w.gn; a.groups_m = w.groups_m; a.grid = w.grid; a.blk4 = w.blk4;
    a.inv_gsz = w.inv_gsz; a.inv_groups_m = w.inv_groups_m; a.inv_gn = w.inv_gn;
    a.inv_tpi = w.inv_tpi; a.inv_tiles_x = w.inv_tiles_x; a.inv_bsz = w.inv_bsz;
}

inline void tile_list(const Walk& a, int th, int tw, std::vector<uint32_t>& t) {
    const int tpi = a.tiles_x * a.tiles_y, gsz = a.gm * a.gn;
    for (int L = 0; L < a.grid; ++L) {
        const int group = L / gsz, within = L % gsz;
        const int gi_n = group / a.groups_m, gi_m = group % a.groups_m;
        const int mt = gi_m * a.gm + within / a.gn, nt = gi_n * a.gn + within % a.gn;
        if (mt >= a.mtiles || nt >= a.ntiles) continue;
        const int b = mt / tpi, trem = mt % tpi;
        int tyi, txi;
        if (!a.blk4) {
            tyi = trem / a.tiles_x; txi = trem % a.tiles_x;
        } else {
            const int bsz = 4 * a.tiles_x, br = trem / bsz, rem = trem % bsz;
            const int rows = std::min(4, a.tiles_y - 4 * br);
            txi = rem / rows; tyi = 4 * br + rem % rows;
        }
        t.push_back((uint32_t)(tyi * th) | (uint32_t)(txi * tw) << 16);
        t.push_back((uint32_t)b | (uint32_t)nt << 16);
    }
}

struct KernelChoice {
    bool ok = false;
    const char* why = nullptr;
    int kernel = K_CONV256;
    int mode = MODE_GEMM1;
    bool fused = false;
    bool mix = false;
    int th = 0, tw = 0;
    int geo = 0;
    int ragged_planes = 0;
    int layout = PK_MAIN;
    int gate = PK_MAIN;
    bool tile_list = false;
    int persist = 0;
};

inline const char* kernel_name(const KernelChoice& ch) {
    if (!ch.ok) return nullptr;
    switch (ch.kernel) {
        case K_CONV256: return ch.mix ? "conv_kernel_mix" : "conv_kernel";
        case K_CONV3W: return ch.fused ? (ch.persist > 0 ? "conv3p" : "conv3w_fused") : "conv3w";
        case K_CONV3P: return "conv3p";
        case K_CONV3S: return ch.fused ? "conv3s_fused" : "conv3s";
        case K_CONV3R: return ch.fused ? "conv3r_fused" : ch.ragged_planes ? "conv3r_ragged" : ch.geo ? "conv3r_8x40" : "conv3r";
        case K_CONV3T: return ch.fused ? "conv3t_fused" : "conv3t";
        case K_MIX16: return "mix16";
        case K_MIX16B: return "mix16b";
    }
    return nullptr;
}

inline int persistent_workgroups(const Knobs& k, int cus) { return k.persist >= 0 ? k.persist : cus; }

inline bool offsets_fit(double planes, double pixels) { return planes * pixels * 16.0 < 4294967296.0; }

struct Conv3Call {
    const LayerPlan* c = nullptr;
    const LayerPlan* mixf = nullptr;
    int epi = EPI_STORE, silu = 0;
    bool film = false;
    int B = 0, H = 0, W = 0, Hout = 0, Wout = 0;
    const void* in = nullptr;
    void* out = nullptr;
    const void* xin = nullptr;
    float alpha = 0.f;
    const void* img = nullptr;
    int R = 0, clamp = 0;
    const ImageViews* views = nullptr;
    const float *gamma = nullptr, *beta = nullptr;
};
inline Conv3Call plain_call(const LayerPlan& c, const void* in, void* out, int B, int H, int W) {
    Conv3Call k;
    k.c = &c; k.in = in; k.out = out; k.B = B; k.H = H; k.W = W;
    return k;
}
inline Conv3Call conv1_call(const LayerPlan& c, const void* in, void* out, int B, int H, int W) {
    Conv3Call k = plain_call(c, in, out, B, H, W);
    k.silu = 1;
    return k;
}
inline Conv3Call d2s_call(const LayerPlan& c, const void* in, void* out, int B, int H, int W, int Hout, int Wout) {
    Conv3Call k = plain_call(c, in, out, B, H, W);
    k.epi = EPI_D2S; k.Hout = Hout; k.Wout = Wout;
    return k;
}
inline Conv3Call head_call(const LayerPlan& c, const void* in, void* out, int B, int H, int W) {
    Conv3Call k = plain_call(c, in, out, B, H, W);
    k.epi = EPI_FINAL; k.Hout = 2 * H; k.Wout = 2 * W;
    return k;
}
inline Conv3Call film_call(const LayerPlan& c, const void* in, void* out, int B, int H, int W, int silu) {
    Conv3Call k = plain_call(c, in, out, B, H, W);
    k.film = true; k.silu = silu;
    return k;
}
template <class Layer> Conv3Call fused_call(const Block<Layer>& b, const void* in, const void* xin, void* out, int B, int H, int W) {
    Conv3Call k = plain_call(b.conv2, in, out, B, H, W);
    k.epi = EPI_FUSEDMIX; k.mixf = &b.mixf; k.xin = xin; k.alpha = b.alpha;
    return k;
}
template <class Layer> Conv3Call conv2_call(const Knobs& k, const Block<Layer>& b, const void* in, const void* xin, int B, int H, int W) {
    return b.fused && k.wide && k.fuse ? fused_call(b, in, xin, nullptr, B, H, W) : plain_call(b.conv2, in, nullptr, B, H, W);
}

inline KernelChoice choose_conv3(const Knobs& k, int dtype, const Conv3Call& call, int cus) {
    KernelChoice ch;
    const LayerPlan& c = *call.c;
    const LayerPlan* mixf = call.mixf;
    const int epi = call.epi, B = call.B, H = call.H, W = call.W;
    const bool fused = epi == EPI_FUSEDMIX;
    const int wgs = persistent_workgroups(k, cus);
    const double px = (double)H * W;
    int mode = MODE_CONV3, th = 8, tw = 32;
    if (c.nt <= 3 && k.wide) {
        const long long waste16 = (long long)((H + 15) / 16 * 16) * ((W + 31) / 32 * 32);
        const long long waste8 = (long long)((H + 7) / 8 * 8) * ((W + 63) / 64 * 64);
        if (waste8 <= waste16) { mode = MODE_C3W8; th = 8; tw = 64; }
        else { mode = MODE_C3W16; th = 16; tw = 32; }
    }
    if (epi == EPI_FINAL && dtype != DT_F32) { mode = MODE_CONV3; th = 8; tw = 32; }
    ch.mode = mode;

    const bool s16 = k.s16 && dtype != DT_F32 && wgs > 0;
    const bool k_fits = c.nchunks32 * 32 * 100 <= c.cp0 * (100 + k.kpad_pct);
    const bool halo_fits = offsets_fit(4, px);
    const int p0 = c.cp0 * dtype_size(dtype) / 16;
    auto listed = [&](int kernel, int lth, int ltw, int layout, int gate) {
        ch.kernel = kernel; ch.fused = fused; ch.th = lth; ch.tw = ltw;
        ch.layout = layout; ch.gate = gate;
        ch.tile_list = true;
        ch.persist = wgs;
        ch.ok = B < 65536 && c.ntiles < 65536 && (H + lth - 1) / lth * lth < 65536 && (W + ltw - 1) / ltw * ltw < 65536;
        if (!ch.ok) ch.why = "tile table: image, batch or N-tile index beyond 16 bits";
        return ch;
    };

    const bool t_fuse = epi == EPI_FUSEDMIX && k.fuse16 && mixf && mixf->has(PK_GATE16T);
    if (k.t && s16 && !call.film && c.has(PK_CONV16T) && c.ntiles == 1 && (c.nchunks32 == 3 || c.nchunks32 >= 6) &&
        (epi == EPI_STORE || t_fuse) && halo_fits && offsets_fit(6, px))
        return listed(K_CONV3T, 12, 64, PK_CONV16T, t_fuse ? PK_GATE16T : PK_MAIN);

    if (k.r && k.r2 && s16 && !call.film && c.nt == 3 && c.has(PK_CONV16) && epi == EPI_STORE && call.silu && c.nchunks32 == 2 && c.cp0 == 48 &&
        halo_fits && offsets_fit(12, px)) {
        ch.ragged_planes = (c.cp0 - 32) / 8;
        return listed(K_CONV3R, 8, 48, PK_CONV16, PK_MAIN);
    }

    if (k.r && k.fuse16 && epi == EPI_FUSEDMIX && s16 && c.nt == 3 && c.ntiles == 1 && c.has(PK_CONV16) && mixf && mixf->has(PK_GATE16R) &&
        mixf->nchunks32 == c.nt && c.nchunks32 >= 6 && p0 % 4 == 0 && k_fits && halo_fits && offsets_fit(12, px))
        return listed(K_CONV3R, 8, 48, PK_CONV16, PK_GATE16R);

    if (k.r && s16 && !call.film && c.nt == 3 && c.has(PK_CONV16) && (epi == EPI_STORE || epi == EPI_D2S) && k_fits && halo_fits &&
        c.nchunks32 >= 3 && p0 % 4 == 0 &&
        (epi == EPI_D2S ? offsets_fit(c.cq_p * dtype_size(dtype) / 16, (double)call.Hout * call.Wout) : offsets_fit(12, px))) {
        const long long rows8 = (long long)((H + 7) / 8 * 8);
        const long long pad48 = rows8 * ((W + 47) / 48 * 48), pad40 = rows8 * ((W + 39) / 40 * 40);
        const long long pads = (long long)((H + th - 1) / th) * th * ((W + tw - 1) / tw) * tw;
        const int geo = pad40 < pad48 ? 1 : 0;
        if ((geo ? pad40 : pad48) <= pads) {
            ch.geo = geo;
            return listed(K_CONV3R, 8, geo ? 40 : 48, PK_CONV16, PK_MAIN);
        }
    }

    ch.th = th; ch.tw = tw;
    ch.fused = fused;
    const bool fuse16 = fused && mixf && mixf->has(PK_GATE16) && k.fuse16 &&
                        mixf->nchunks32 == c.nt;
    if (mode != MODE_CONV3 && (epi == EPI_STORE || epi == EPI_D2S || fuse16) && wgs > 0) {
        const int tiles_x = (W + tw - 1) / tw, tiles_y = (H + th - 1) / th;
        const Walk g = pick_order(tiles_x, tiles_y, B * tiles_x * tiles_y, c.ntiles, (double)pack_bytes(c, PK_MAIN),
                                  (double)B * H * W * c.cp0 * (double)dtype_size(dtype), k);
        if (s16 && c.has(PK_CONV16) && k_fits && halo_fits) {
            ch.layout = PK_CONV16;
            ch.gate = fused ? PK_GATE16 : PK_MAIN;
            ch.persist = wgs;
        } else if (g.grid > wgs && offsets_fit(2, px)) {
            ch.persist = wgs;
        }
    }
    if (call.film && ch.layout == PK_MAIN) {
        ch.why = "the FiLM epilogue exists on the 16x16x32 kernel only: bf16 / fp16, at most 96 output channels per "
                 "N tile, input channels within 12.5 % of a multiple of 32";
        return ch;
    }
    ch.kernel = mode == MODE_CONV3 ? K_CONV256 : ch.persist == 0 || (fused && ch.layout == PK_MAIN) ? K_CONV3W : ch.layout != PK_MAIN ? K_CONV3S : K_CONV3P;
    ch.ok = true;
    return ch;
}

inline KernelChoice choose_mix(const Knobs& k, int dtype, const LayerPlan& c, int B, int H, int W, int cus) {
    KernelChoice ch;
    ch.ok = ch.mix = true;
    ch.mode = MODE_GEMM1;
    const bool mix16 = c.has(PK_MIX16) && offsets_fit(c.cp0 * dtype_size(dtype) / 16.0, (double)B * H * W);
    const int wgs = k.persist > 0 ? k.persist : cus;
    if (mix16 && k.mix16b && c.has(PK_MIX16B) && wgs > 0) {
        ch.kernel = K_MIX16B; ch.layout = PK_MIX16B; ch.persist = wgs;
    } else if (mix16) {
        ch.kernel = K_MIX16; ch.layout = PK_MIX16;
    } else {
        ch.kernel = K_CONV256;
    }
    return ch;
}

inline const LayerPlan* plan_debug_layer(BlockPlan& b, int dtype, int op, int cin, int cout, Refusal* why) {
    switch (op) {
        case 0: case 1: case 2: case 3: case 4: case 5:
            plan_conv(b.conv1, dtype, MODE_CONV3, cout, cin, 3, 3, op == 2 ? OUT_D2S : op == 3 ? OUT_FINAL : OUT_PLAIN, SRC_PLAIN, 0, 0);
            return &b.conv1;
        case 6: case 8:
            plan_block(b, dtype, cout, cin);
            if (op == 6) return &b.conv2;
            if (b.fused) return &b.mixf;
            *why = refuse(MZ_ERR_INVALID_ARGUMENT, "the block does not fuse conv2 and the mix");
            return nullptr;
        case 7:
            if (cin == 2 * cout) {
                plan_conv(b.mix, dtype, MODE_GEMM1, cout, cin, 1, 1, OUT_PLAIN, SRC_CONCAT, cout, cout);
                return &b.mix;
            }
            *why = refuse(MZ_ERR_INVALID_ARGUMENT, "a mix has cin = 2 cout");
            return nullptr;
    }
    *why = refuse(MZ_ERR_INVALID_ARGUMENT, "bad op %d", op);
    return nullptr;
}

}
```

Measured before the change: 707.8 MPix/s.

## Pair output-channel tiles per pixel tile in conv3r to reuse the input halo

Adds a paired variant of the conv3r kernel for three-chunk layers with several output-channel tiles. Each workgroup walks all output-channel tiles of one pixel tile in sequence, so the input halo is loaded once and kept in a fixed LDS slot instead of being reloaded for every channel tile. A new pixel-major tile list and a three-slot LDS layout support this, and it is on by default with an environment knob to turn it off. It cuts global halo traffic, at the cost of extra LDS and a more complex schedule that may hurt load balance or the overlap of loads with compute.

```diff
diff --git a/include/mewzoom_hip.h b/include/mewzoom_hip.h
--- a/include/mewzoom_hip.h
+++ b/include/mewzoom_hip.h
@@ -150,6 +150,8 @@
 
 int mz_debug_tile_list(int B, int tiles_y, int tiles_x, int ntiles, int gm, int gn, int blk4, int th, int tw, unsigned int* out, int cap);
 
+int mz_debug_pair_walk(int B, int tiles_y, int tiles_x, int ntiles, int blk4, int th, int tw, int wgs, unsigned int* out, int cap);
+
 const char* mz_debug_select(int dtype, int op, int cin, int cout, int B, int H, int W, int cus);
 
 typedef struct mz_debug_step {
diff --git a/ultrazoom_amd/csrc/mz_conv3r.h b/ultrazoom_amd/csrc/mz_conv3r.h
--- a/ultrazoom_amd/csrc/mz_conv3r.h
+++ b/ultrazoom_amd/csrc/mz_conv3r.h
@@ -161,7 +161,9 @@
 
 }
 
-template <class TT, int NSEG, int EPI, bool SILU, int GEO = 0, bool RAG = false>
+enum { PK_NONE = 0, PK_FIRST = 1, PK_MIDDLE = 2, PK_LAST = 3 };
+
+template <class TT, int NSEG, int EPI, bool SILU, int GEO = 0, bool RAG = false, bool PAIR = false>
 __global__ __launch_bounds__(512) void conv3r_kernel(const ConvArgs a) {
     using namespace r3;
     using namespace relay;
@@ -172,8 +174,10 @@
     constexpr bool FUSE = EPI == EPI_FUSEDMIX;
     static_assert(!FUSE || GEO == 0, "the fused variant is built for the 8 x 48 tile");
     constexpr int B_SLOT = S::SLOT;
+    constexpr int B_BASE = PAIR ? 3 * A_SLOT : r3::B_BASE;
     static_assert(!FUSE || NSEG == 3, "the gate weights need the LDS that three weight segments leave free");
     static_assert(!RAG || (NSEG == 3 && EPI == EPI_STORE && GEO == 0), "the ragged two-chunk variant: three steps per chunk, plain stores, 8 x 48 tiles");
+    static_assert(!PAIR || (NSEG == 3 && !FUSE && !RAG), "the paired variant: three steps per chunk, plain / SiLU / sub-pixel stores");
     extern __shared__ __attribute__((aligned(16))) char smem[];
     const int w = __builtin_amdgcn_readfirstlane((int)threadIdx.x >> 6);
     const int team = w >> 2, wq = w & 3;
@@ -194,8 +198,19 @@
         return TileE{e[0], e[1]};
     };
     int a_pos = pos;
+    [[maybe_unused]] int a_n = 0, c_pos = pos, c_n = 0;
+    [[maybe_unused]] const int ntl = a.ntiles;
     TileE eD, eA, eB;
-    auto advance = [&]() __attribute__((always_inline)) { a_pos += step; };
+    auto advance = [&]() __attribute__((always_inline)) {
+        if constexpr (PAIR) {
+            if (++a_n == ntl) { a_n = 0; a_pos += step; }
+        } else {
+            a_pos += step;
+        }
+    };
+    [[maybe_unused]] auto seq_inc = [&](int& p, int& n) __attribute__((always_inline)) {
+        if (++n == ntl) { n = 0; p += step; }
+    };
     auto tile_origin = [&](const TileE e, int& b, int& y0, int& x0) __attribute__((always_inline)) {
         b = (int)(e.bn & 0xffffu);
         y0 = (int)(e.yx & 0xffffu);
@@ -439,21 +454,24 @@
     const char* wA = nullptr;
     const char* wB = nullptr;
     bool okB = false;
-    auto loader_step = [&](auto wk_tag, auto es_tag, auto en_tag, auto sg_tag, auto last_tag, int k) __attribute__((always_inline)) {
+    auto loader_step = [&](auto wk_tag, auto es_tag, auto en_tag, auto sg_tag, auto last_tag, auto kind_tag, int k) __attribute__((always_inline)) {
+        constexpr int KIND = decltype(kind_tag)::value;
+        static_assert(PAIR == (KIND != PK_NONE), "the paired kernel's steps say which tile of its pixel tile they serve");
         constexpr int WK = decltype(wk_tag)::value;
         constexpr int ES = decltype(es_tag)::value, EN = WK == 0 ? 0 : decltype(en_tag)::value, sg = decltype(sg_tag)::value;
         constexpr bool last = decltype(last_tag)::value != 0;
+        constexpr bool HALO_STEP = sg == 0 && (!PAIR || (KIND == PK_FIRST && !last) || (KIND == PK_LAST && last));
         [[maybe_unused]] constexpr int rs_c = 1 + (EN > 0 ? 2 : 0) + (sg == 0 ? 0 : 1);
         static_assert(EN <= 3, "three output registers");
         constexpr int VM_AFTER0 = WK == 1 ? EN : (WK == 2 ? (ES + 1 < NPF ? NF : 0) : (WK == 4 ? EN * NT : 0));
-        constexpr int VM_AFTER = VM_AFTER0 + (NSEG == 3 && sg == 0 ? 8 : 0);
+        constexpr int VM_AFTER = VM_AFTER0 + (NSEG == 3 && HALO_STEP ? 8 : 0);
         RS_BEGIN();
         if constexpr (WK == 2 && ES == 0) fuse_x(ic<0>{});
         if constexpr (WK == 3) x_landed(ic<ES>{});
         constexpr bool HALO_LATE = NSEG == 3;
         auto halo_image = [&]() __attribute__((always_inline)) {
             const __amdgpu_buffer_rsrc_t h_rsrc = halo_rsrc(last ? 0 : k + 1);
-            uint32_t h_off = (uint32_t)(us ^ 1) * (uint32_t)A_SLOT;
+            uint32_t h_off = PAIR ? (uint32_t)(last ? 0 : k + 1) * (uint32_t)A_SLOT : (uint32_t)(us ^ 1) * (uint32_t)A_SLOT;
             asm volatile("" : "+s"(h_off));
             char* const h_dst = smem + h_off;
             const bool rag = RAG && !last && k + 2 == nchunks;
@@ -482,7 +500,7 @@
             if constexpr (WP > 6) wseg_piece(ic<6>{}, wsrc, w_pieces, w_dst, lo);
             static_assert(WP <= 7, "seven weight pieces per wave and step");
         }
-        if constexpr (sg == 0 && HALO_LATE) halo_image();
+        if constexpr (HALO_STEP && HALO_LATE) halo_image();
         __builtin_amdgcn_sched_barrier(0);
         asm volatile("" ::: "memory");
         RS_LAP(4 * rs_c);
@@ -507,8 +525,8 @@
         if constexpr (sg == NSEG - 1) {
             if constexpr (last) {
                 if constexpr (FUSE) zero_acc(acc);
-                prime(next3(hs), us ^ 1);
-            } else {
+                prime(next3(hs), PAIR ? 0 : us ^ 1);
+            } else if constexpr (!PAIR) {
                 if (k + 2 == nchunks && okB) {
                     set_load_tile(eB);
                 }
@@ -522,47 +540,61 @@
         RS_LAP(4 * rs_c + 3);
         RS_COUNT(20 + rs_c);
         hs = next3(hs);
-        if constexpr (sg == NSEG - 1) us ^= 1;
-    };
-    auto loader_chunk = [&](auto e0_tag, auto n0_tag, auto n1_tag, auto last_tag, int k) __attribute__((always_inline)) {
+        if constexpr (sg == NSEG - 1 && !PAIR) us ^= 1;
+    };
+    auto loader_chunk = [&](auto e0_tag, auto n0_tag, auto n1_tag, auto last_tag, auto kind_tag, int k) __attribute__((always_inline)) {
         constexpr int E0 = decltype(e0_tag)::value < NE ? decltype(e0_tag)::value : NE;
         constexpr int N0 = decltype(n0_tag)::value < NE - E0 ? decltype(n0_tag)::value : NE - E0;
         constexpr int N1 = decltype(n1_tag)::value < NE - E0 - N0 ? decltype(n1_tag)::value : NE - E0 - N0;
         if constexpr (NSEG == 2) {
-            loader_step(ic<(N0 > 0)>{}, ic<E0>{}, ic<N0>{}, ic<0>{}, last_tag, k);
-            loader_step(ic<(N1 > 0)>{}, ic<E0 + N0>{}, ic<N1>{}, ic<1>{}, last_tag, k);
+            loader_step(ic<(N0 > 0)>{}, ic<E0>{}, ic<N0>{}, ic<0>{}, last_tag, kind_tag, k);
+            loader_step(ic<(N1 > 0)>{}, ic<E0 + N0>{}, ic<N1>{}, ic<1>{}, last_tag, kind_tag, k);
         } else {
             constexpr int N1a = N1 / 2, N1b = N1 - N1a;
-            loader_step(ic<(N0 > 0)>{}, ic<E0>{}, ic<N0>{}, ic<0>{}, last_tag, k);
-            loader_step(ic<(N1a > 0)>{}, ic<E0 + N0>{}, ic<N1a>{}, ic<1>{}, last_tag, k);
-            loader_step(ic<(N1b > 0)>{}, ic<E0 + N0 + N1a>{}, ic<N1b>{}, ic<2>{}, last_tag, k);
+            loader_step(ic<(N0 > 0)>{}, ic<E0>{}, ic<N0>{}, ic<0>{}, last_tag, kind_tag, k);
+            loader_step(ic<(N1a > 0)>{}, ic<E0 + N0>{}, ic<N1a>{}, ic<1>{}, last_tag, kind_tag, k);
+            loader_step(ic<(N1b > 0)>{}, ic<E0 + N0 + N1a>{}, ic<N1b>{}, ic<2>{}, last_tag, kind_tag, k);
         }
     };
     auto fuse_chunk = [&](auto p0_tag, auto g_tag, auto last_tag, int k) __attribute__((always_inline)) {
         static_assert(!FUSE || NSEG == 3, "the fused variant runs three steps per chunk");
-        loader_step(ic<2>{}, p0_tag, g_tag, ic<0>{}, last_tag, k);
-        loader_step(ic<3>{}, p0_tag, g_tag, ic<1>{}, last_tag, k);
-        loader_step(ic<4>{}, p0_tag, g_tag, ic<NSEG - 1>{}, last_tag, k);
-    };
-    auto plain_chunks = [&](int k0) __attribute__((always_inline)) {
-        for (int k = k0; k + 1 < nchunks; ++k) loader_chunk(ic<0>{}, ic<0>{}, ic<0>{}, ic<0>{}, k);
-        loader_chunk(ic<0>{}, ic<0>{}, ic<0>{}, ic<1>{}, nchunks - 1);
-    };
-    auto loader_phase = [&](auto epi_tag) __attribute__((always_inline)) {
+        loader_step(ic<2>{}, p0_tag, g_tag, ic<0>{}, last_tag, ic<PK_NONE>{}, k);
+        loader_step(ic<3>{}, p0_tag, g_tag, ic<1>{}, last_tag, ic<PK_NONE>{}, k);
+        loader_step(ic<4>{}, p0_tag, g_tag, ic<NSEG - 1>{}, last_tag, ic<PK_NONE>{}, k);
+    };
+    auto plain_chunks = [&](auto kind_tag, int k0) __attribute__((always_inline)) {
+        using KT = decltype(kind_tag);
+        for (int k = k0; k + 1 < nchunks; ++k) loader_chunk(ic<0>{}, ic<0>{}, ic<0>{}, ic<0>{}, KT{}, k);
+        loader_chunk(ic<0>{}, ic<0>{}, ic<0>{}, ic<1>{}, KT{}, nchunks - 1);
+    };
+    auto loader_phase = [&](auto epi_tag, auto kind_tag) __attribute__((always_inline)) {
         constexpr bool DO_EPI = decltype(epi_tag)::value != 0;
+        using KT = decltype(kind_tag);
+        constexpr int KIND = KT::value;
         wA = wsrc_of(tile_nt(eA));
-        okB = a_pos + step < cnt;
+        if constexpr (PAIR && KIND != PK_LAST) okB = true;
+        else okB = a_pos + step < cnt;
         wB = wsrc_of(tile_nt(okB ? eB : eA));
-        const TileE eA2 = tile_at(a_pos + 2 * step), eB2 = tile_at(a_pos + 3 * step);
+        TileE eA2, eB2;
+        if constexpr (PAIR) {
+            int p2 = c_pos, n2 = c_n;
+            seq_inc(p2, n2);
+            eA2 = tile_at(c_pos);
+            eB2 = tile_at(p2);
+        } else {
+            eA2 = tile_at(a_pos + 2 * step);
+            eB2 = tile_at(a_pos + 3 * step);
+        }
         if constexpr (DO_EPI) {
             RS_BEGIN();
-            set_load_tile(eA);
+            if constexpr (!PAIR || KIND == PK_FIRST) set_load_tile(eA);
+            else if constexpr (KIND == PK_LAST) set_load_tile(okB ? eB : eA);
             epi_setup();
             RS_FENCE();
             RS_LAP(27);
             if constexpr (RAG) {
-                loader_chunk(ic<0>{}, ic<3>{}, ic<6>{}, ic<0>{}, 0);
-                loader_chunk(ic<9>{}, ic<3>{}, ic<6>{}, ic<1>{}, 1);
+                loader_chunk(ic<0>{}, ic<3>{}, ic<6>{}, ic<0>{}, KT{}, 0);
+                loader_chunk(ic<9>{}, ic<3>{}, ic<6>{}, ic<1>{}, KT{}, 1);
             } else if constexpr (FUSE) {
                 fuse_chunk(ic<0>{}, ic<1>{}, ic<0>{}, 0);
                 fuse_chunk(ic<1>{}, ic<1>{}, ic<0>{}, 1);
@@ -573,35 +605,49 @@
                     fuse_chunk(ic<5>{}, ic<1>{}, ic<1>{}, 5);
                 } else {
                     fuse_chunk(ic<5>{}, ic<1>{}, ic<0>{}, 5);
-                    plain_chunks(6);
+                    plain_chunks(KT{}, 6);
                 }
+            } else if constexpr (PAIR) {
+                loader_chunk(ic<0>{}, ic<2>{}, ic<4>{}, ic<0>{}, KT{}, 0);
+                loader_chunk(ic<6>{}, ic<2>{}, ic<4>{}, ic<0>{}, KT{}, 1);
+                loader_chunk(ic<12>{}, ic<2>{}, ic<4>{}, ic<1>{}, KT{}, 2);
             } else if (nchunks >= 6) {
-                loader_chunk(ic<0>{}, ic<1>{}, ic<2>{}, ic<0>{}, 0);
-                loader_chunk(ic<3>{}, ic<1>{}, ic<2>{}, ic<0>{}, 1);
-                loader_chunk(ic<6>{}, ic<1>{}, ic<2>{}, ic<0>{}, 2);
-                loader_chunk(ic<9>{}, ic<1>{}, ic<2>{}, ic<0>{}, 3);
-                loader_chunk(ic<12>{}, ic<1>{}, ic<2>{}, ic<0>{}, 4);
+                loader_chunk(ic<0>{}, ic<1>{}, ic<2>{}, ic<0>{}, KT{}, 0);
+                loader_chunk(ic<3>{}, ic<1>{}, ic<2>{}, ic<0>{}, KT{}, 1);
+                loader_chunk(ic<6>{}, ic<1>{}, ic<2>{}, ic<0>{}, KT{}, 2);
+                loader_chunk(ic<9>{}, ic<1>{}, ic<2>{}, ic<0>{}, KT{}, 3);
+                loader_chunk(ic<12>{}, ic<1>{}, ic<2>{}, ic<0>{}, KT{}, 4);
                 if (nchunks == 6) {
-                    loader_chunk(ic<15>{}, ic<1>{}, ic<2>{}, ic<1>{}, 5);
+                    loader_chunk(ic<15>{}, ic<1>{}, ic<2>{}, ic<1>{}, KT{}, 5);
                 } else {
-                    loader_chunk(ic<15>{}, ic<1>{}, ic<2>{}, ic<0>{}, 5);
-                    plain_chunks(6);
+                    loader_chunk(ic<15>{}, ic<1>{}, ic<2>{}, ic<0>{}, KT{}, 5);
+                    plain_chunks(KT{}, 6);
                 }
             } else {
                 constexpr int F3 = NSEG == 3 ? 2 : 3;
-                loader_chunk(ic<0>{}, ic<F3>{}, ic<6 - F3>{}, ic<0>{}, 0);
-                loader_chunk(ic<6>{}, ic<F3>{}, ic<6 - F3>{}, ic<0>{}, 1);
+                loader_chunk(ic<0>{}, ic<F3>{}, ic<6 - F3>{}, ic<0>{}, KT{}, 0);
+                loader_chunk(ic<6>{}, ic<F3>{}, ic<6 - F3>{}, ic<0>{}, KT{}, 1);
                 if (nchunks == 3) {
-                    loader_chunk(ic<12>{}, ic<F3>{}, ic<6 - F3>{}, ic<1>{}, 2);
+                    loader_chunk(ic<12>{}, ic<F3>{}, ic<6 - F3>{}, ic<1>{}, KT{}, 2);
                 } else {
-                    loader_chunk(ic<12>{}, ic<F3>{}, ic<6 - F3>{}, ic<0>{}, 2);
-                    plain_chunks(3);
+                    loader_chunk(ic<12>{}, ic<F3>{}, ic<6 - F3>{}, ic<0>{}, KT{}, 2);
+                    plain_chunks(KT{}, 3);
                 }
             }
-        } else {
-            plain_chunks(0);
+        } else if constexpr (PAIR) {
+            loader_chunk(ic<0>{}, ic<0>{}, ic<0>{}, ic<0>{}, KT{}, 0);
+            loader_chunk(ic<0>{}, ic<0>{}, ic<0>{}, ic<0>{}, KT{}, 1);
+            loader_chunk(ic<0>{}, ic<0>{}, ic<0>{}, ic<1>{}, KT{}, 2);
+        } else {
+            plain_chunks(KT{}, 0);
         }
         eD = eB; eA = eA2; eB = eB2;
+        if constexpr (PAIR) {
+            eA.bn |= (uint32_t)c_n << 16;
+            seq_inc(c_pos, c_n);
+            eB.bn |= (uint32_t)c_n << 16;
+            seq_inc(c_pos, c_n);
+        }
         asm volatile("" ::"s"(eA.yx), "s"(eA.bn), "s"(eB.yx), "s"(eB.bn));
     };
 
@@ -610,8 +656,8 @@
         const int g = lane_ >> 4, c = lane_ & 15;
         const uint32_t a_lane = lds_base + g * A_PLANE + ((2 * wq) * ROWW + c) * 16;
         Bases bs;
-        bs.a_cur = a_lane + us * A_SLOT;
-        bs.a_nxt = a_lane + (us ^ 1) * A_SLOT;
+        bs.a_cur = a_lane + (PAIR ? 0 : us) * A_SLOT;
+        bs.a_nxt = a_lane + (PAIR ? 1 : us ^ 1) * A_SLOT;
         const uint32_t a_str = (uint32_t)((c >= 8 ? ROWW - 8 : 32) * 16);
         bs.a2_cur = bs.a_cur + a_str;
         bs.a2_nxt = bs.a_nxt + a_str;
@@ -634,8 +680,13 @@
                 groups<TT, NSEG, GEO, S::start(2), S::start(3), XP>(acc, f, bs, false);
                 step_tail();
             }
-            const uint32_t v_ = bs.a_cur; bs.a_cur = bs.a_nxt; bs.a_nxt = v_;
-            if constexpr (GEO == 1) { const uint32_t v2_ = bs.a2_cur; bs.a2_cur = bs.a2_nxt; bs.a2_nxt = v2_; }
+            if constexpr (PAIR) {
+                const uint32_t v_ = bs.a_cur; bs.a_cur = bs.a_nxt; bs.a_nxt = XP == 0 ? v_ + 2u * A_SLOT : v_ - (uint32_t)A_SLOT;
+                if constexpr (GEO == 1) { const uint32_t v2_ = bs.a2_cur; bs.a2_cur = bs.a2_nxt; bs.a2_nxt = XP == 0 ? v2_ + 2u * A_SLOT : v2_ - (uint32_t)A_SLOT; }
+            } else {
+                const uint32_t v_ = bs.a_cur; bs.a_cur = bs.a_nxt; bs.a_nxt = v_;
+                if constexpr (GEO == 1) { const uint32_t v2_ = bs.a2_cur; bs.a2_cur = bs.a2_nxt; bs.a2_nxt = v2_; }
+            }
         };
         RS_BEGIN();
         int kc = 0;
@@ -655,7 +706,7 @@
         RS_COUNT(1);
         const int adv = (NSEG * nchunks) % 3;
         hs = hs + adv >= 3 ? hs + adv - 3 : hs + adv;
-        us ^= nchunks & 1;
+        if constexpr (!PAIR) us ^= nchunks & 1;
     };
     auto final_fuse_pf = [&](auto pf_tag) __attribute__((always_inline)) {
         constexpr int pf = decltype(pf_tag)::value;
@@ -678,8 +729,16 @@
     };
 
     if (team == 1) {
-        eA = tile_at(a_pos);
-        eB = tile_at(a_pos + step);
+        if constexpr (PAIR) {
+            eA = tile_at(c_pos);
+            seq_inc(c_pos, c_n);
+            eB = tile_at(c_pos);
+            eB.bn |= (uint32_t)c_n << 16;
+            seq_inc(c_pos, c_n);
+        } else {
+            eA = tile_at(a_pos);
+            eB = tile_at(a_pos + step);
+        }
         eD = eA;
         wA = wsrc_of(tile_nt(eA));
         set_load_tile(eA);
@@ -707,13 +766,24 @@
         wait_vmcnt<0>();
         __builtin_amdgcn_s_barrier();
         if constexpr (FUSE) zero_acc(acc);
-        loader_phase(ic<0>{});
+        loader_phase(ic<0>{}, ic<(PAIR ? PK_FIRST : PK_NONE)>{});
         advance();
         if (a_pos >= cnt) { RS_DUMP(); return; }
     } else {
-        eD = tile_at(a_pos);
-        eA = tile_at(a_pos + step);
-        eB = tile_at(a_pos + 2 * step);
+        if constexpr (PAIR) {
+            eD = tile_at(c_pos);
+            seq_inc(c_pos, c_n);
+            eA = tile_at(c_pos);
+            eA.bn |= (uint32_t)c_n << 16;
+            seq_inc(c_pos, c_n);
+            eB = tile_at(c_pos);
+            eB.bn |= (uint32_t)c_n << 16;
+            seq_inc(c_pos, c_n);
+        } else {
+            eD = tile_at(a_pos);
+            eA = tile_at(a_pos + step);
+            eB = tile_at(a_pos + 2 * step);
+        }
         asm volatile("" ::"s"(eD.yx), "s"(eD.bn), "s"(eA.yx), "s"(eA.bn), "s"(eB.yx), "s"(eB.bn));
         __builtin_amdgcn_s_barrier();
         if constexpr (FUSE) zero_acc(acc);
@@ -729,7 +799,13 @@
             RS_DUMP();
             return;
         }
-        loader_phase(ic<1>{});
+        if constexpr (PAIR) {
+            if (a_n == 0) loader_phase(ic<1>{}, ic<PK_FIRST>{});
+            else if (a_n + 1 == ntl) loader_phase(ic<1>{}, ic<PK_LAST>{});
+            else loader_phase(ic<1>{}, ic<PK_MIDDLE>{});
+        } else {
+            loader_phase(ic<1>{}, ic<PK_NONE>{});
+        }
         advance();
         if (a_pos >= cnt) { RS_DUMP(); return; }
     }
diff --git a/ultrazoom_amd/csrc/mz_conv3r.hip b/ultrazoom_amd/csrc/mz_conv3r.hip
--- a/ultrazoom_amd/csrc/mz_conv3r.hip
+++ b/ultrazoom_amd/csrc/mz_conv3r.hip
@@ -10,7 +10,19 @@
     constexpr size_t lds = r3::Seg<NSEG>::lds_bytes(EPI == EPI_FUSEDMIX);
     return launch_lds<conv3r_kernel<TT, NSEG, EPI, SILU, GEO, RAG>>(a.persist, 512, lds, a, s);
 }
+template <class TT, int EPI, bool SILU = false> static hipError_t r_launch_pair(const ConvArgs& a, hipStream_t s) {
+    constexpr size_t lds = 3 * r3::A_SLOT + 3 * r3::Seg<3>::SLOT;
+    return launch_lds<conv3r_kernel<TT, 3, EPI, SILU, 0, false, true>>(a.persist, 512, lds, a, s);
+}
 template <class TT> static hipError_t r_epi(const ConvArgs& a, hipStream_t s) {
+    if (a.pair) {
+        if (a.nchunks16 != 3 || a.ntiles < 2 || a.ragged_planes || a.geo != 0) return hipErrorInvalidValue;
+        switch (a.epi) {
+            case EPI_STORE: return a.silu ? r_launch_pair<TT, EPI_STORE, true>(a, s) : r_launch_pair<TT, EPI_STORE>(a, s);
+            case EPI_D2S: return r_launch_pair<TT, EPI_D2S>(a, s);
+            default: return hipErrorInvalidValue;
+        }
+    }
     if (a.ragged_planes) {
         if (a.nchunks16 != 2 || a.ragged_planes < 1 || a.ragged_planes > 3 || a.epi != EPI_STORE || !a.silu || a.geo != 0) return hipErrorInvalidValue;
         return r_launch<TT, 3, EPI_STORE, true, 0, true>(a, s);
diff --git a/ultrazoom_amd/csrc/mz_debug.cpp b/ultrazoom_amd/csrc/mz_debug.cpp
--- a/ultrazoom_amd/csrc/mz_debug.cpp
+++ b/ultrazoom_amd/csrc/mz_debug.cpp
@@ -44,6 +44,17 @@
     tile_list(group_walk(tiles_x, tiles_y, mtiles, ntiles, std::min(gm, mtiles), std::min(gn, ntiles), blk4 ? 1 : 0), th, tw, t);
     const int n = (int)(t.size() / 2);
     for (int i = 0; i < n && i < cap; ++i) { out[2 * i] = t[2 * i]; out[2 * i + 1] = t[2 * i + 1]; }
+    return n;
+}
+
+extern "C" int mz_debug_pair_walk(int B, int tiles_y, int tiles_x, int ntiles, int blk4, int th, int tw, int wgs, unsigned int* out, int cap) {
+    if (B < 1 || tiles_x < 1 || tiles_y < 1 || ntiles < 2 || th < 1 || tw < 1 || wgs < 8 || (wgs & 7) || !out || cap < 0) return MZ_ERR_INVALID_ARGUMENT;
+    const int mtiles = B * tiles_x * tiles_y;
+    std::vector<uint32_t> t;
+    pair_walk_list(group_walk(tiles_x, tiles_y, mtiles, ntiles, 1, 1, blk4 ? 1 : 0), th, tw, wgs, t);
+    const int n = (int)(t.size() / 4);
+    for (int i = 0; i < n && i < cap; ++i)
+        for (int j = 0; j < 4; ++j) out[4 * i + j] = t[4 * i + j];
     return n;
 }
 
diff --git a/ultrazoom_amd/csrc/mz_kernels.h b/ultrazoom_amd/csrc/mz_kernels.h
--- a/ultrazoom_amd/csrc/mz_kernels.h
+++ b/ultrazoom_amd/csrc/mz_kernels.h
@@ -74,6 +74,7 @@
     int view;
     long long vin[4], vout[4];
     int win_y0, win_x0, win_h, win_w;
+    int pair;
 };
 
 struct ImageViews {
diff --git a/ultrazoom_amd/csrc/mz_plan.h b/ultrazoom_amd/csrc/mz_plan.h
--- a/ultrazoom_amd/csrc/mz_plan.h
+++ b/ultrazoom_amd/csrc/mz_plan.h
@@ -19,8 +19,10 @@
     int blk4 = 1;
     int r = 1;
     int r2 = 1;
+    int pair = 1;
     int t = 1;
 };
+inline bool pair_knob() { return getenv("MZ_NO_PAIR") == nullptr; }
 inline Knobs read_knobs() {
     Knobs k;
     k.wide = getenv("MZ_NO_WIDE") == nullptr;
@@ -31,6 +33,7 @@
     k.r = getenv("MZ_NO_R") == nullptr;
     k.t = getenv("MZ_NO_T") == nullptr;
     k.r2 = getenv("MZ_NO_R2") == nullptr;
+    k.pair = pair_knob();
     k.blk4 = getenv("MZ_NO_BLK4") == nullptr;
     if (const char* e = getenv("MZ_KPAD_PCT")) k.kpad_pct = atoi(e);
     if (getenv("MZ_NO_PERSIST") != nullptr) k.persist = 0;
diff --git a/ultrazoom_amd/csrc/mz_runner.h b/ultrazoom_amd/csrc/mz_runner.h
--- a/ultrazoom_amd/csrc/mz_runner.h
+++ b/ultrazoom_amd/csrc/mz_runner.h
@@ -201,7 +201,8 @@
             a.nchunks16 = pack_shape(c, ch.layout).nchunks;
             if (fused) a.wmix16 = weights(k.mixf).packed[ch.gate].p;
         }
-        if (ch.tile_list) tile_table(a, w, ch.th, ch.tw, ch.persist);
+        a.pair = ch.pair ? 1 : 0;
+        if (ch.tile_list) tile_table(a, ch.pair ? pixel_walk(w) : w, ch.th, ch.tw, ch.persist);
         if (rc) return;
         a.persist = std::min((a.grid + 7) / 8 * 8, ch.persist);
         a.film_gamma = k.gamma; a.film_beta = k.beta;
diff --git a/ultrazoom_amd/csrc/mz_select.h b/ultrazoom_amd/csrc/mz_select.h
--- a/ultrazoom_amd/csrc/mz_select.h
+++ b/ultrazoom_amd/csrc/mz_select.h
@@ -78,6 +78,28 @@
     }
 }
 
+inline Walk pixel_walk(const Walk& w) { return group_walk(w.tiles_x, w.tiles_y, w.mtiles, 1, 1, 1, w.blk4); }
+
+inline void pair_walk_list(const Walk& w, int th, int tw, int wgs, std::vector<uint32_t>& t) {
+    std::vector<uint32_t> px;
+    tile_list(pixel_walk(w), th, tw, px);
+    const int grid = (int)(px.size() / 2), launched = std::min((grid + 7) / 8 * 8, wgs), step = launched >> 3;
+    const int q = grid >> 3, rem = grid & 7;
+    for (int wg = 0; wg < launched; ++wg) {
+        const int xcd = wg & 7, pos = wg >> 3;
+        const int cnt = q + (xcd < rem ? 1 : 0);
+        const int base = xcd < rem ? xcd * (q + 1) : rem * (q + 1) + (xcd - rem) * q;
+        uint32_t seq = 0;
+        for (int p = pos; p < cnt; p += step)
+            for (int nt = 0; nt < w.ntiles; ++nt) {
+                t.push_back(px[2 * (size_t)(base + p)]);
+                t.push_back(px[2 * (size_t)(base + p) + 1] | (uint32_t)nt << 16);
+                t.push_back((uint32_t)wg);
+                t.push_back(seq++);
+            }
+    }
+}
+
 struct KernelChoice {
     bool ok = false;
     const char* why = nullptr;
@@ -88,11 +110,15 @@
     int th = 0, tw = 0;
     int geo = 0;
     int ragged_planes = 0;
+    bool pair = false;
+    bool unpaired = false;
     int layout = PK_MAIN;
     int gate = PK_MAIN;
     bool tile_list = false;
     int persist = 0;
 };
+
+inline const char* unpaired_name() { return "conv3r_unpaired"; }
 
 inline const char* kernel_name(const KernelChoice& ch) {
     if (!ch.ok) return nullptr;
@@ -101,7 +127,7 @@
         case K_CONV3W: return ch.fused ? (ch.persist > 0 ? "conv3p" : "conv3w_fused") : "conv3w";
         case K_CONV3P: return "conv3p";
         case K_CONV3S: return ch.fused ? "conv3s_fused" : "conv3s";
-        case K_CONV3R: return ch.fused ? "conv3r_fused" : ch.ragged_planes ? "conv3r_ragged" : ch.geo ? "conv3r_8x40" : "conv3r";
+        case K_CONV3R: return ch.fused ? "conv3r_fused" : ch.ragged_planes ? "conv3r_ragged" : ch.geo ? "conv3r_8x40" : ch.unpaired ? unpaired_name() : "conv3r";
         case K_CONV3T: return ch.fused ? "conv3t_fused" : "conv3t";
         case K_MIX16: return "mix16";
         case K_MIX16B: return "mix16b";
@@ -218,6 +244,9 @@
         const int geo = pad40 < pad48 ? 1 : 0;
         if ((geo ? pad40 : pad48) <= pads) {
             ch.geo = geo;
+            const bool pairs = c.nchunks32 == 3 && c.ntiles >= 2 && geo == 0;
+            ch.pair = pairs && k.pair;
+            ch.unpaired = pairs && !k.pair;
             return listed(K_CONV3R, 8, geo ? 40 : 48, PK_CONV16, PK_MAIN);
         }
     }
```

After: 709.1 MPix/s, median of 6. No clear change (+0.2%).
